# bacchus-snu/bacchus-gpu-controller

Hardware: AMD Instinct MI355X
Metric: reconcile p99 (ms) + admission p50 (ms); CR apply→Ready/sec on 8×MI355X node (higher is better)
Workload: dtype none

## Files before the change

native/apiserver/server.cc:

```cpp
#include "apiserver/server.h"

#include <algorithm>
#include <array>
#include <atomic>
#include <chrono>
#include <condition_variable>
#include <deque>
#include <functional>
#include <iterator>
#include <mutex>
#include <optional>
#include <regex>
#include <set>
#include <sstream>
#include <thread>
#include <unordered_map>
#include <unordered_set>

#include <openssl/crypto.h>

#include "apiserver/fieldset.h"
#include "core/crypto.h"
#include "core/http.h"
#include "core/json_patch.h"
#include "core/log.h"
#include "core/metrics.h"
#include "core/process.h"
#include "core/stall.h"
#include "core/trace.h"
#include "core/net.h"
#include "core/yaml.h"
#include "crd/schema.h"
#include "kube/leader.h"
#include "kube/quantity.h"
#include "kube/resource.h"

namespace bgc::apiserver {

using json::Value;
using kube::ResourceType;

namespace {


struct StatusError : std::runtime_error {
  int code;
  std::string reason;
  Value details;
  StatusError(int c, std::string r, const std::string& msg, Value d = {})
      : std::runtime_error(msg), code(c), reason(std::move(r)), details(std::move(d)) {}
};

Value status_body(int code, const std::string& reason, const std::string& message, const Value& details = {}) {
  Value s = Value::object({{"kind", "Status"}, {"apiVersion", "v1"}, {"metadata", Value::object()},
                           {"status", code < 400 ? "Success" : "Failure"}, {"message", message},
                           {"reason", reason}});
  if (!details.is_null()) s["details"] = details;
  s["code"] = code;
  return s;
}

std::string resource_ref(const ResourceType& rt) {
  return rt.group.empty() ? rt.plural : rt.plural + "." + rt.group;
}

StatusError not_found(const ResourceType& rt, const std::string& name) {
  return StatusError(404, "NotFound", resource_ref(rt) + " \"" + name + "\" not found",
                     Value::object({{"name", name}, {"group", rt.group}, {"kind", rt.plural}}));
}

StatusError already_exists(const ResourceType& rt, const std::string& name) {
  return StatusError(409, "AlreadyExists", resource_ref(rt) + " \"" + name + "\" already exists",
                     Value::object({{"name", name}, {"group", rt.group}, {"kind", rt.plural}}));
}

StatusError conflict(const ResourceType& rt, const std::string& name) {
  return StatusError(409, "Conflict",
                     "Operation cannot be fulfilled on " + resource_ref(rt) + " \"" + name +
                         "\": the object has been modified; please apply your changes to the latest version and try again",
                     Value::object({{"name", name}, {"group", rt.group}, {"kind", rt.plural}}));
}

StatusError invalid(const ResourceType& rt, const std::string& name, const std::string& msg) {
  return StatusError(422, "Invalid", rt.kind + "." + rt.group + " \"" + name + "\" is invalid: " + msg,
                     Value::object({{"name", name}, {"group", rt.group}, {"kind", rt.kind}}));
}

std::string now_rfc3339() {
  std::string s = kube::rfc3339_micro_now();
  return s.substr(0, 19) + "Z";
}

bool dns1123_label(const std::string& s) {
  if (s.empty() || s.size() > 63) return false;
  for (size_t i = 0; i < s.size(); ++i) {
    char c = s[i];
    bool ok = (c >= 'a' && c <= 'z') || (c >= '0' && c <= '9') || (c == '-' && i != 0 && i + 1 != s.size());
    if (!ok) return false;
  }
  return true;
}

bool dns1123_subdomain(const std::string& s) {
  if (s.empty() || s.size() > 253) return false;
  size_t start = 0;
  while (true) {
    size_t dot = s.find('.', start);
    std::string part = s.substr(start, dot == std::string::npos ? std::string::npos : dot - start);
    if (!dns1123_label(part)) return false;
    if (dot == std::string::npos) return true;
    start = dot + 1;
  }
}


struct Requirement {
  std::string key;
  std::string op;
  std::vector<std::string> values;
};

std::string trim(std::string s) {
  while (!s.empty() && s.front() == ' ') s.erase(0, 1);
  while (!s.empty() && s.back() == ' ') s.pop_back();
  return s;
}

std::vector<Requirement> parse_selector(const std::string& sel) {
  std::vector<Requirement> out;
  std::vector<std::string> parts;
  int depth = 0;
  std::string cur;
  for (char c : sel) {
    if (c == '(') ++depth;
    if (c == ')') --depth;
    if (c == ',' && depth == 0) {
      parts.push_back(cur);
      cur.clear();
    } else {
      cur.push_back(c);
    }
  }
  if (!cur.empty()) parts.push_back(cur);
  for (auto p : parts) {
    p = trim(p);
    if (p.empty()) continue;
    Requirement r;
    size_t pos;
    if (p[0] == '!') {
      r.key = trim(p.substr(1));
      r.op = "!exists";
    } else if ((pos = p.find(" notin ")) != std::string::npos || (pos = p.find(" in ")) != std::string::npos) {
      bool notin = p.compare(pos, 7, " notin ") == 0;
      r.key = trim(p.substr(0, pos));
      r.op = notin ? "notin" : "in";
      size_t lp = p.find('('), rp = p.rfind(')');
      if (lp == std::string::npos || rp == std::string::npos) throw StatusError(400, "BadRequest", "invalid selector: " + p);
      std::string inner = p.substr(lp + 1, rp - lp - 1);
      std::stringstream ss(inner);
      std::string v;
      while (std::getline(ss, v, ',')) r.values.push_back(trim(v));
    } else if ((pos = p.find("!=")) != std::string::npos) {
      r.key = trim(p.substr(0, pos));
      r.op = "!=";
      r.values.push_back(trim(p.substr(pos + 2)));
    } else if ((pos = p.find("==")) != std::string::npos) {
      r.key = trim(p.substr(0, pos));
      r.op = "=";
      r.values.push_back(trim(p.substr(pos + 2)));
    } else if ((pos = p.find('=')) != std::string::npos) {
      r.key = trim(p.substr(0, pos));
      r.op = "=";
      r.values.push_back(trim(p.substr(pos + 1)));
    } else {
      r.key = p;
      r.op = "exists";
    }
    out.push_back(r);
  }
  return out;
}

bool selector_matches(const std::vector<Requirement>& reqs, const Value& obj) {
  const Value& labels = obj.get("metadata").get("labels");
  for (const auto& r : reqs) {
    const Value* v = labels.find(r.key);
    bool has = v && v->is_string();
    std::string val = has ? v->as_string() : "";
    if (r.op == "exists" && !has) return false;
    if (r.op == "!exists" && has) return false;
    if (r.op == "=" && (!has || val != r.values[0])) return false;
    if (r.op == "!=" && has && val == r.values[0]) return false;
    if (r.op == "in" && (!has || std::find(r.values.begin(), r.values.end(), val) == r.values.end())) return false;
    if (r.op == "notin" && has && std::find(r.values.begin(), r.values.end(), val) != r.values.end()) return false;
  }
  return true;
}

struct FieldFilter {
  std::string name, ns;
  std::string name_prefix;
  bool name_ok(std::string_view n) const {
    return (name.empty() || n == name) && (name_prefix.empty() || n.substr(0, name_prefix.size()) == name_prefix);
  }
};

FieldFilter parse_field_selector(const std::string& s) {
  FieldFilter f;
  std::stringstream ss(s);
  std::string part;
  while (std::getline(ss, part, ',')) {
    size_t eq = part.find('=');
    if (eq == std::string::npos) continue;
    std::string k = trim(part.substr(0, eq));
    std::string v = trim(part.substr(part[eq + 1] == '=' ? eq + 2 : eq + 1));
    if (k == "metadata.name") f.name = v;
    else if (k == "metadata.namespace") f.ns = v;
    else if (k == "kube-lite.test/name-prefix") f.name_prefix = v;
  }
  return f;
}


struct UserInfo {
  std::string username;
  std::string uid;
  std::vector<std::string> groups;
  bool is_admin() const { return std::find(groups.begin(), groups.end(), "system:masters") != groups.end(); }
  Value to_json() const {
    Value g = Value::array();
    for (auto& x : groups) g.push_back(x);
    Value v = Value::object({{"username", username}});
    if (!uid.empty()) v["uid"] = uid;
    v["groups"] = g;
    return v;
  }
};

struct TypeStore;

struct TypeInfo {
  ResourceType rt;
  std::shared_ptr<const Value> schema;
  bool custom = false;
  std::shared_ptr<TypeStore> store;
  std::string key() const { return rt.group + "/" + rt.version + "/" + rt.plural; }
};

struct ManagerEntry {
  std::string operation;
  std::string api_version;
  std::string time;
  std::string subresource;
  FieldSet fields;
  bool operator==(const ManagerEntry& o) const {
    return operation == o.operation && fields == o.fields && subresource == o.subresource;
  }
};
using Managers = std::map<std::string, ManagerEntry>;

inline const std::shared_ptr<const Managers>& no_managers() {
  static const std::shared_ptr<const Managers> empty = std::make_shared<const Managers>();
  return empty;
}

struct Stored {
  std::shared_ptr<const Value> obj;
  uint64_t rv = 0;
  std::weak_ptr<const std::string> line;
  std::shared_ptr<const Managers> managers = no_managers();
};

bool wants_metadata(const http::Request& req) {
  const std::string* a = req.headers.get("Accept");
  return a && a->find("as=PartialObjectMetadata") != std::string::npos;
}

void dump_partial_metadata(const Value& obj, std::string& out) {
  out += "{\"kind\":\"PartialObjectMetadata\",\"apiVersion\":\"meta.k8s.io/v1\",\"metadata\":";
  obj.get("metadata").dump_to(out);
  out += "}";
}

std::string partial_metadata_line(const std::string& line) {
  std::string_view body(line);
  while (!body.empty() && (body.back() == '\n' || body.back() == '\r')) body.remove_suffix(1);
  const std::string_view type = json::raw_member(body, "type");
  const std::string_view md = json::raw_member(json::raw_member(body, "object"), "metadata");
  std::string out;
  out.reserve(md.size() + 128);
  out += "{\"type\":";
  out.append(type.data(), type.size());
  out += ",\"object\":{\"kind\":\"PartialObjectMetadata\",\"apiVersion\":\"meta.k8s.io/v1\",\"metadata\":";
  if (md.empty()) out += "{}";
  else out.append(md.data(), md.size());
  out += "}}\n";
  return out;
}

enum class View : uint8_t { AsIs, Added, Deleted };

struct EventRec {
  uint64_t rv;
  std::string type_key;
  std::string ns;
  std::shared_ptr<const Value> meta;
  std::shared_ptr<const std::string> line;
  struct Transitions {
    std::shared_ptr<const Value> prev_meta;
    std::shared_ptr<const std::string> prev_line;
    std::once_flag added_once, deleted_once;
    std::string added, added_meta, deleted, deleted_meta;
  };
  std::unique_ptr<Transitions> tr;
  const std::string& metadata_line() const {
    std::call_once(meta_once_, [this] { meta_line_ = partial_metadata_line(*line); });
    return meta_line_;
  }
  const std::string& line_as(View v, bool meta_only) const {
    if (v == View::AsIs || !tr) return meta_only ? metadata_line() : *line;
    Transitions& t = *tr;
    if (v == View::Added) {
      std::call_once(t.added_once, [&] {
        t.added = retyped_line(*line, "ADDED");
        t.added_meta = partial_metadata_line(t.added);
      });
      return meta_only ? t.added_meta : t.added;
    }
    std::call_once(t.deleted_once, [&] {
      t.deleted = deleted_from_prev();
      t.deleted_meta = partial_metadata_line(t.deleted);
    });
    return meta_only ? t.deleted_meta : t.deleted;
  }

 private:
  static std::string retyped_line(const std::string& l, const char* type) {
    const std::string_view t = json::raw_member(l, "type");
    std::string out;
    if (t.empty()) return l;
    out.reserve(l.size() + 8);
    out.append(l, 0, static_cast<size_t>(t.data() - l.data()));
    out += '"';
    out += type;
    out += '"';
    out.append(t.data() + t.size(), l.data() + l.size());
    return out;
  }
  std::string deleted_from_prev() const {
    std::string_view prev(*tr->prev_line);
    while (!prev.empty() && (prev.back() == '\n' || prev.back() == '\r')) prev.remove_suffix(1);
    const std::string_view obj = json::raw_member(prev, "object");
    const std::string_view old_rv = json::raw_member(json::raw_member(obj, "metadata"), "resourceVersion");
    const std::string_view new_rv =
        json::raw_member(json::raw_member(json::raw_member(*line, "object"), "metadata"), "resourceVersion");
    std::string out = "{\"type\":\"DELETED\",\"object\":";
    if (old_rv.empty()) {
      out.append(obj.data(), obj.size());
    } else {
      out.append(obj.data(), static_cast<size_t>(old_rv.data() - obj.data()));
      out.append(new_rv.data(), new_rv.size());
      out.append(old_rv.data() + old_rv.size(), obj.data() + obj.size());
    }
    out += "}\n";
    return out;
  }
  mutable std::once_flag meta_once_;
  mutable std::string meta_line_;
};

struct QueuedEvent {
  std::shared_ptr<const EventRec> e;
  View view = View::AsIs;
};

std::shared_ptr<const Value> filter_view(const Value& obj) {
  const Value& m = obj.get("metadata");
  Value meta = Value::object({{"name", m.get("name")}});
  if (m.contains("labels")) meta["labels"] = m.get("labels");
  return std::make_shared<const Value>(Value::object({{"metadata", std::move(meta)}}));
}

struct WatchSub {
  std::string type_key;
  std::string ns;
  std::vector<Requirement> sel;
  FieldFilter fields;
  std::mutex m;
  std::condition_variable cv;
  std::deque<QueuedEvent> q;
  bool closed = false;
  bool overflow = false;

  void close() {
    {
      std::lock_guard<std::mutex> g(m);
      closed = true;
    }
    cv.notify_one();
  }
};

class RwLock {
 public:
  RwLock() {
    const char* kind = std::getenv("BGC_KL_RWLOCK");
    mutex_only_ = !kind || (std::string(kind) != "writer" && std::string(kind) != "reader");
    pthread_rwlockattr_t a;
    pthread_rwlockattr_init(&a);
    pthread_rwlockattr_setkind_np(&a, kind && std::string(kind) == "reader" ? PTHREAD_RWLOCK_PREFER_READER_NP
                                                                           : PTHREAD_RWLOCK_PREFER_WRITER_NONRECURSIVE_NP);
    pthread_rwlock_init(&l_, &a);
    pthread_rwlockattr_destroy(&a);
  }
  ~RwLock() { pthread_rwlock_destroy(&l_); }
  RwLock(const RwLock&) = delete;
  RwLock& operator=(const RwLock&) = delete;
  void lock() {
    if (mutex_only_) m_.lock();
    else pthread_rwlock_wrlock(&l_);
  }
  bool try_lock() { return mutex_only_ ? m_.try_lock() : pthread_rwlock_trywrlock(&l_) == 0; }
  void unlock() {
    if (mutex_only_) m_.unlock();
    else pthread_rwlock_unlock(&l_);
  }
  void lock_shared() {
    if (mutex_only_) m_.lock();
    else pthread_rwlock_rdlock(&l_);
  }
  bool try_lock_shared() { return mutex_only_ ? m_.try_lock() : pthread_rwlock_tryrdlock(&l_) == 0; }
  void unlock_shared() { unlock(); }

 private:
  pthread_rwlock_t l_;
  std::mutex m_;
  bool mutex_only_ = false;
};

thread_local std::vector<std::shared_ptr<WatchSub>> t_pending_wakeups;
thread_local std::vector<std::shared_ptr<const EventRec>> t_retired_events;

inline void flush_watch_wakeups() {
  for (auto& w : t_pending_wakeups) w->cv.notify_one();
  t_pending_wakeups.clear();
  t_retired_events.clear();
}

struct LockStats {
  std::atomic<uint64_t> acquisitions{0}, shared{0}, contended{0}, wait_ns{0}, hold_ns{0};
};

class StoreLock {
 public:
  StoreLock(RwLock& m, LockStats& st, LockStats* also = nullptr) : m_(m), st_(st), also_(also) {
    if (!m_.try_lock()) {
      int64_t t0 = metrics::now_ns();
      m_.lock();
      const auto waited = static_cast<uint64_t>(metrics::now_ns() - t0);
      st_.contended.fetch_add(1, std::memory_order_relaxed);
      st_.wait_ns.fetch_add(waited, std::memory_order_relaxed);
      if (also_) {
        also_->contended.fetch_add(1, std::memory_order_relaxed);
        also_->wait_ns.fetch_add(waited, std::memory_order_relaxed);
      }
    }
    t_acq_ = metrics::now_ns();
  }
  ~StoreLock() {
    const auto held = static_cast<uint64_t>(metrics::now_ns() - t_acq_);
    st_.acquisitions.fetch_add(1, std::memory_order_relaxed);
    st_.hold_ns.fetch_add(held, std::memory_order_relaxed);
    if (also_) {
      also_->acquisitions.fetch_add(1, std::memory_order_relaxed);
      also_->hold_ns.fetch_add(held, std::memory_order_relaxed);
    }
    m_.unlock();
    flush_watch_wakeups();
  }
  StoreLock(const StoreLock&) = delete;
  StoreLock& operator=(const StoreLock&) = delete;

 private:
  RwLock& m_;
  LockStats& st_;
  LockStats* also_;
  int64_t t_acq_ = 0;
};

class SharedStoreLock {
 public:
  SharedStoreLock(RwLock& m, LockStats& st) : m_(m) {
    if (!m_.try_lock_shared()) {
      int64_t t0 = metrics::now_ns();
      m_.lock_shared();
      st.contended.fetch_add(1, std::memory_order_relaxed);
      st.wait_ns.fetch_add(static_cast<uint64_t>(metrics::now_ns() - t0), std::memory_order_relaxed);
    }
    st.shared.fetch_add(1, std::memory_order_relaxed);
  }
  ~SharedStoreLock() { m_.unlock_shared(); }
  SharedStoreLock(const SharedStoreLock&) = delete;
  SharedStoreLock& operator=(const SharedStoreLock&) = delete;

 private:
  RwLock& m_;
};

struct TypeStore {
  struct Shard {
    RwLock mu;
    std::unordered_map<std::string, Stored> objs;
  };
  class Shards {
   public:
    explicit Shards(size_t n) : n_(std::max<size_t>(1, n)), p_(new Shard[n_]) {}
    Shard* begin() { return p_.get(); }
    Shard* end() { return p_.get() + n_; }
    std::reverse_iterator<Shard*> rbegin() { return std::reverse_iterator<Shard*>(end()); }
    std::reverse_iterator<Shard*> rend() { return std::reverse_iterator<Shard*>(begin()); }
    size_t size() const { return n_; }
    Shard& operator[](size_t i) { return p_[i]; }

   private:
    size_t n_;
    std::unique_ptr<Shard[]> p_;
  };
  explicit TypeStore(size_t n_shards) : shards(n_shards) {}
  Shards shards;
  Shard& shard(const std::string& key) {
    return shards.size() == 1 ? shards[0] : shards[std::hash<std::string>{}(key) % shards.size()];
  }
  RwLock seq;
  std::atomic<uint64_t> version{0};
  LockStats stats;
  LockStats seq_stats;
  std::deque<std::shared_ptr<const EventRec>> history;
  uint64_t compacted_rv = 0;
  std::mutex watches_mu;
  std::set<std::shared_ptr<WatchSub>> watches;
};

class AllShards {
 public:
  AllShards(TypeStore& ts, bool exclusive) : ts_(ts), exclusive_(exclusive) {
    for (auto& sh : ts_.shards) {
      if (exclusive_) {
        if (!sh.mu.try_lock()) {
          const int64_t t0 = metrics::now_ns();
          sh.mu.lock();
          ts_.stats.contended.fetch_add(1, std::memory_order_relaxed);
          ts_.stats.wait_ns.fetch_add(static_cast<uint64_t>(metrics::now_ns() - t0), std::memory_order_relaxed);
        }
      } else if (!sh.mu.try_lock_shared()) {
        const int64_t t0 = metrics::now_ns();
        sh.mu.lock_shared();
        ts_.stats.contended.fetch_add(1, std::memory_order_relaxed);
        ts_.stats.wait_ns.fetch_add(static_cast<uint64_t>(metrics::now_ns() - t0), std::memory_order_relaxed);
      }
    }
    ts_.stats.acquisitions.fetch_add(1, std::memory_order_relaxed);
  }
  ~AllShards() {
    for (auto it = ts_.shards.rbegin(); it != ts_.shards.rend(); ++it) {
      if (exclusive_) it->mu.unlock();
      else it->mu.unlock_shared();
    }
    flush_watch_wakeups();
  }
  AllShards(const AllShards&) = delete;
  AllShards& operator=(const AllShards&) = delete;

 private:
  TypeStore& ts_;
  bool exclusive_;
};

struct FaultRule {
  std::string method;
  std::regex path;
  std::string path_src;
  int status = 0;
  int retry_after_s = -1;
  int delay_ms = 0;
  int hold_ms = 0;
  int remaining = -1;
  bool reset = false;
  std::string message;
};

struct ParsedPath {
  TypeInfo* ti = nullptr;
  std::string ns;
  std::string name;
  std::string sub;
  bool collection = false;
};

thread_local std::string t_trace_tag;
thread_local std::string t_trace_name;

void trace_step(const std::string& name, const char* step) {
  if (!t_trace_tag.empty()) trace::mark(name, t_trace_tag + step);
}

struct WriteResult {
  std::shared_ptr<const Value> obj;
  int code = 200;
  std::shared_ptr<const std::string> line;
  std::string_view body() const {
    static const std::string kPrefixEnd = ",\"object\":";
    if (!line) return {};
    size_t at = line->find(kPrefixEnd);
    if (at == std::string::npos || line->size() < at + kPrefixEnd.size() + 2) return {};
    at += kPrefixEnd.size();
    return std::string_view(*line).substr(at, line->size() - at - 2);
  }
};

std::string obj_key(const ResourceType& rt, const std::string& ns, const std::string& name) { return rt.key(ns, name); }

}


struct ApiServer::Impl {
  Options opts;
  std::unique_ptr<http::Server> server;

  RwLock types_mu;
  std::map<std::string, TypeInfo> types;
  std::atomic<uint64_t> rv{1000};
  std::mutex index_mu;
  std::unordered_map<std::string, std::pair<std::string, std::string>> by_uid;
  using Ref = std::pair<std::string, std::string>;
  struct RefHash {
    size_t operator()(const Ref& r) const { return std::hash<std::string>{}(r.first) * 31 + std::hash<std::string>{}(r.second); }
  };
  std::unordered_map<std::string, std::unordered_set<Ref, RefHash>> by_owner;
  std::unordered_map<std::string, std::unordered_set<Ref, RefHash>> by_namespace;

  struct GcItem {
    bool is_namespace = false;
    std::string id;
    bool finish_namespace = false;
  };
  std::mutex gc_mu;
  std::condition_variable gc_cv;
  std::deque<GcItem> gc_queue;
  bool gc_stop = false;
  std::atomic<uint64_t> gc_collected{0};
  std::vector<std::thread> gc_threads;

  std::unordered_map<std::string, UserInfo> tokens;

  std::mutex fault_mu;
  std::vector<FaultRule> faults;

  struct ListSnapshot {
    uint64_t rv = 0;
    std::vector<std::shared_ptr<const Value>> items;
    std::chrono::steady_clock::time_point expires;
  };
  std::mutex list_mu;
  std::map<uint64_t, ListSnapshot> list_snapshots;
  uint64_t next_list_id = 1;
  std::atomic<uint64_t> list_pages{0};

  static constexpr uint64_t kRvMask = 0x5bd1e9955bd1e995ULL;
  std::string rv_str(uint64_t v) const {
    if (!opts.opaque_rv) return std::to_string(v);
    static const char* digits = "0123456789abcdefghijklmnopqrstuvwxyz";
    uint64_t x = v ^ kRvMask;
    std::string out;
    do {
      out.insert(out.begin(), digits[x % 36]);
      x /= 36;
    } while (x);
    return "kl." + out;
  }
  bool parse_rv(const std::string& s, uint64_t* v) const {
    if (!opts.opaque_rv) {
      if (s.empty() || s.find_first_not_of("0123456789") != std::string::npos) return false;
      *v = std::strtoull(s.c_str(), nullptr, 10);
      return true;
    }
    if (s.rfind("kl.", 0) != 0 || s.size() < 4) return false;
    uint64_t x = 0;
    for (size_t i = 3; i < s.size(); ++i) {
      const char c = s[i];
      int d = c >= '0' && c <= '9' ? c - '0' : c >= 'a' && c <= 'z' ? c - 'a' + 10 : -1;
      if (d < 0) return false;
      x = x * 36 + static_cast<uint64_t>(d);
    }
    *v = x ^ kRvMask;
    return true;
  }

  std::mutex hook_mu;
  struct FastHook {
    std::shared_ptr<const Value> cfg;
    std::shared_ptr<http::Client> client;
    std::string path;
  };
  std::map<const Value*, FastHook> hook_fast;
  std::map<std::string, std::shared_ptr<http::Client>> hook_clients;
  std::atomic<bool> webhook_h2{false};
  std::atomic<int64_t> write_latency_us{0};
  std::atomic<int> watch_coalesce_us{0};

  std::atomic<uint64_t> requests{0};
  std::atomic<uint64_t> faults_hit{0};
  LockStats types_stats;

  explicit Impl(Options o) : opts(std::move(o)) {
    if (const char* e = std::getenv("BGC_KL_STORE_SHARDS"); e && *e) opts.store_shards = std::max(1, std::atoi(e));
    watch_coalesce_us = opts.watch_coalesce_us;
    if (const char* e = std::getenv("BGC_KL_H2_CALLER_READS"); e && *e) opts.webhook_h2_caller_reads = std::string(e) != "0";
    webhook_h2 = opts.webhook_http2;
    write_latency_us = opts.write_latency_us;
    for (const ResourceType* rt : kube::types::builtin()) {
      TypeInfo ti;
      ti.rt = *rt;
      ti.store = std::make_shared<TypeStore>(opts.store_shards);
      types[ti.key()] = ti;
    }
    if (!opts.token_file.empty()) load_tokens(opts.token_file);
    const TypeInfo& ns_ti = types.at(kube::types::Namespace.group + "/" + kube::types::Namespace.version + "/" +
                                     kube::types::Namespace.plural);
    for (const char* name : {"default", "kube-system", "kube-public", "kube-node-lease"}) {
      const uint64_t v = ++rv;
      Value ns = Value::object(
          {{"apiVersion", "v1"}, {"kind", "Namespace"},
           {"metadata", Value::object({{"name", name}, {"uid", crypto::uuid_v4()}, {"creationTimestamp", now_rfc3339()},
                                       {"resourceVersion", rv_str(v)}})},
           {"spec", Value::object({{"finalizers", Value::array({Value("kubernetes")})}})},
           {"status", Value::object({{"phase", "Active"}})}});
      Stored st;
      st.obj = std::make_shared<const Value>(std::move(ns));
      st.rv = v;
      ns_ti.store->shard(obj_key(ns_ti.rt, "", name)).objs[obj_key(ns_ti.rt, "", name)] = std::move(st);
    }
    for (int i = 0; i < std::max(1, opts.gc_workers); ++i) gc_threads.emplace_back([this] {
      gc_loop();
      OPENSSL_thread_stop();
    });
  }

  ~Impl() {
    {
      std::lock_guard<std::mutex> g(gc_mu);
      gc_stop = true;
    }
    gc_cv.notify_all();
    for (auto& t : gc_threads) t.join();
  }

  template <typename F>
  void for_each_store(F f) {
    std::vector<std::pair<std::string, std::shared_ptr<TypeStore>>> stores;
    {
      SharedStoreLock lk(types_mu, types_stats);
      for (auto& [k, ti] : types) stores.emplace_back(k, ti.store);
    }
    for (auto& [k, st] : stores) f(k, *st);
  }

  TypeInfo* type_by_key(const std::string& key) {
    SharedStoreLock lk(types_mu, types_stats);
    auto it = types.find(key);
    return it == types.end() ? nullptr : &it->second;
  }

  void load_tokens(const std::string& path) {
    std::stringstream ss(net::read_file(path));
    std::string line;
    while (std::getline(ss, line)) {
      if (line.empty() || line[0] == '#') continue;
      std::vector<std::string> cols;
      std::string cur;
      bool q = false;
      for (char c : line) {
        if (c == '"') {
          q = !q;
          continue;
        }
        if (c == ',' && !q) {
          cols.push_back(cur);
          cur.clear();
          continue;
        }
        cur.push_back(c);
      }
      cols.push_back(cur);
      if (cols.size() < 2) continue;
      UserInfo u;
      u.username = cols[1];
      if (cols.size() > 2) u.uid = cols[2];
      if (cols.size() > 3 && !cols[3].empty()) {
        std::stringstream gs(cols[3]);
        std::string g;
        while (std::getline(gs, g, ',')) u.groups.push_back(g);
      }
      u.groups.push_back("system:authenticated");
      tokens[cols[0]] = u;
    }
  }

  UserInfo authenticate(const http::Request& req) {
    UserInfo u;
    std::string auth = req.headers.get_or("Authorization");
    if (auth.rfind("Bearer ", 0) == 0) {
      auto it = tokens.find(auth.substr(7));
      if (it == tokens.end()) throw StatusError(401, "Unauthorized", "Unauthorized");
      u = it->second;
    } else if (!req.peer_cn.empty()) {
      u.username = req.peer_cn;
      u.groups = req.peer_orgs;
      u.groups.push_back("system:authenticated");
    } else if (opts.anonymous_admin) {
      u.username = "system:admin";
      u.groups = {"system:masters", "system:authenticated"};
    } else {
      throw StatusError(401, "Unauthorized", "Unauthorized");
    }
    if (const std::string* imp = req.headers.get("Impersonate-User")) {
      if (!u.is_admin()) {
        throw StatusError(403, "Forbidden", "users \"" + *imp + "\" is forbidden: User \"" + u.username +
                                                "\" cannot impersonate resource \"users\" in API group \"\" at the cluster scope");
      }
      UserInfo imp_u;
      imp_u.username = *imp;
      for (const auto& kv : req.headers.items()) {
        std::string lk = kv.first;
        for (auto& c : lk) c = static_cast<char>(std::tolower(static_cast<unsigned char>(c)));
        if (lk == "impersonate-group") {
          std::stringstream gs(kv.second);
          std::string g;
          while (std::getline(gs, g, ',')) {
            if (!trim(g).empty()) imp_u.groups.push_back(trim(g));
          }
        }
      }
      imp_u.groups.push_back("system:authenticated");
      u = imp_u;
    }
    return u;
  }

  TypeInfo* find_type(const std::string& group, const std::string& version, const std::string& plural) {
    auto it = types.find(group + "/" + version + "/" + plural);
    return it == types.end() ? nullptr : &it->second;
  }

  bool parse_path(const std::string& path, ParsedPath& out, std::string& group, std::string& version,
                  std::vector<std::string>& rest) {
    std::vector<std::string> segs;
    std::stringstream ss(path);
    std::string s;
    while (std::getline(ss, s, '/')) {
      if (!s.empty()) segs.push_back(s);
    }
    size_t i = 0;
    if (segs.size() >= 2 && segs[0] == "api") {
      group = "";
      version = segs[1];
      i = 2;
    } else if (segs.size() >= 3 && segs[0] == "apis") {
      group = segs[1];
      version = segs[2];
      i = 3;
    } else {
      return false;
    }
    rest.assign(segs.begin() + static_cast<long>(i), segs.end());
    if (rest.empty()) return false;
    SharedStoreLock lk(types_mu, types_stats);
    if (rest[0] == "namespaces" && rest.size() >= 3) {
      TypeInfo* ti = find_type(group, version, rest[2]);
      if (ti && ti->rt.namespaced) {
        out.ti = ti;
        out.ns = rest[1];
        out.collection = rest.size() == 3;
        if (rest.size() >= 4) out.name = rest[3];
        if (rest.size() >= 5) out.sub = rest[4];
        return true;
      }
    }
    TypeInfo* ti = find_type(group, version, rest[0]);
    if (!ti) throw StatusError(404, "NotFound", "the server could not find the requested resource");
    out.ti = ti;
    out.collection = rest.size() == 1;
    if (rest.size() >= 2) out.name = rest[1];
    if (rest.size() >= 3) out.sub = rest[2];
    return true;
  }

  struct PreparedEvent {
    std::string head, tail;
    bool ok = false;
    std::shared_ptr<const Value> filter;
    std::shared_ptr<EventRec> rec;
  };

  std::shared_ptr<const std::string> emit_locked(const TypeInfo& ti, const std::string& ns, uint64_t ev_rv,
                                                 std::string line, std::shared_ptr<const Value> filter,
                                                 std::shared_ptr<EventRec> rec) {
    TypeStore& st = *ti.store;
    st.version.fetch_add(1, std::memory_order_release);
    if (!rec) rec = std::make_shared<EventRec>();
    rec->rv = ev_rv;
    rec->type_key = ti.key();
    rec->ns = ns;
    rec->meta = std::move(filter);
    rec->line = std::make_shared<const std::string>(std::move(line));
    st.history.push_back(rec);
    while (st.history.size() > opts.history_limit) {
      st.compacted_rv = st.history.front()->rv;
      t_retired_events.push_back(std::move(st.history.front()));
      st.history.pop_front();
    }
    const std::string& name = rec->meta->get("metadata").get_string("name");
    std::lock_guard<std::mutex> wg(st.watches_mu);
    for (const auto& w : st.watches) {
      if (!w->ns.empty() && w->ns != ns) continue;
      if (!w->fields.name_ok(name)) continue;
      View view;
      if (!view_for(w->sel, *rec, &view)) continue;
      {
        std::lock_guard<std::mutex> g(w->m);
        if (w->q.size() > 100000) w->overflow = true;
        else w->q.push_back({rec, view});
      }
      t_pending_wakeups.push_back(w);
    }
    return rec->line;
  }

  static bool view_for(const std::vector<Requirement>& sel, const EventRec& e, View* view) {
    *view = View::AsIs;
    if (sel.empty()) return true;
    const bool now_in = selector_matches(sel, *e.meta);
    if (!e.tr) return now_in;
    const bool was_in = selector_matches(sel, *e.tr->prev_meta);
    if (now_in && !was_in) *view = View::Added;
    else if (!now_in && was_in) *view = View::Deleted;
    return now_in || was_in;
  }

  struct HookMatch {
    std::string name;
    std::shared_ptr<const Value> cfg;
    const Value* hook;
  };
  std::mutex hook_match_mu;
  uint64_t hook_match_version = ~uint64_t{0};
  std::unordered_map<std::string, std::vector<HookMatch>> hook_match_cache;

  std::vector<HookMatch> matching_webhooks(const TypeInfo& ti, const std::string& sub, const std::string& op) {
    TypeInfo* mwc = type_by_key(kube::types::MutatingWebhookConfiguration.group + "/v1/mutatingwebhookconfigurations");
    if (!mwc) return {};
    const std::string cache_key = ti.key() + "|" + sub + "|" + op;
    {
      std::lock_guard<std::mutex> g(hook_match_mu);
      if (hook_match_version == mwc->store->version.load(std::memory_order_acquire)) {
        auto it = hook_match_cache.find(cache_key);
        if (it != hook_match_cache.end()) return it->second;
      }
    }
    std::vector<HookMatch> out;
    AllShards lk(*mwc->store, false);
    const uint64_t version = mwc->store->version.load(std::memory_order_acquire);
    std::string res = ti.rt.plural + (sub.empty() ? "" : "/" + sub);
    for (auto& sh : mwc->store->shards)
    for (auto& kv : sh.objs) {
      for (const auto& hook : kv.second.obj->get("webhooks").items()) {
        for (const auto& rule : hook.get("rules").items()) {
          auto contains = [](const Value& arr, const std::string& v) {
            for (const auto& x : arr.items()) {
              if (x.is_string() && (x.as_string() == "*" || x.as_string() == v)) return true;
            }
            return false;
          };
          bool res_ok = false;
          for (const auto& r : rule.get("resources").items()) {
            std::string rs = r.as_string();
            if (rs == res || rs == "*/*" || (rs == "*" && sub.empty()) ||
                (sub.size() && rs == "*/" + sub) || (rs == ti.rt.plural + "/*")) {
              res_ok = true;
            }
          }
          if (contains(rule.get("apiGroups"), ti.rt.group) && contains(rule.get("apiVersions"), ti.rt.version) &&
              contains(rule.get("operations"), op) && res_ok) {
            out.push_back({hook.get_string("name"), kv.second.obj, &hook});
            break;
          }
        }
      }
    }
    {
      std::lock_guard<std::mutex> g(hook_match_mu);
      if (hook_match_version != version) {
        hook_match_cache.clear();
        hook_match_version = version;
      }
      hook_match_cache[cache_key] = out;
    }
    return out;
  }

  std::shared_ptr<http::Client> hook_client(const HookMatch& hm, std::string& path_out) {
    {
      std::lock_guard<std::mutex> lk(hook_mu);
      auto it = hook_fast.find(hm.hook);
      if (it != hook_fast.end()) {
        path_out = it->second.path;
        return it->second.client;
      }
    }
    auto c = hook_client_slow(*hm.hook, path_out);
    std::lock_guard<std::mutex> lk(hook_mu);
    if (hook_fast.size() > 256) hook_fast.clear();
    hook_fast[hm.hook] = {hm.cfg, c, path_out};
    return c;
  }

  std::shared_ptr<http::Client> hook_client_slow(const Value& hook, std::string& path_out) {
    const Value& cc = hook.get("clientConfig");
    std::string ca = cc.get_string("caBundle");
    std::string base, server_name;
    if (cc.get("url").is_string()) {
      http::Url u = http::parse_url(cc.get_string("url"));
      base = u.scheme + "://" + u.host + ":" + std::to_string(u.port);
      path_out = u.path.empty() ? "/" : u.path;
    } else {
      const Value& svc = cc.get("service");
      std::string ns = svc.get_string("namespace"), name = svc.get_string("name");
      int port = svc.get("port").is_int() ? static_cast<int>(svc.get("port").as_int()) : 443;
      path_out = svc.get_string("path", "/");
      server_name = name + "." + ns + ".svc";
      auto ov = opts.service_overrides.find(ns + "/" + name);
      std::string hostport = ov != opts.service_overrides.end() ? ov->second : server_name + ":" + std::to_string(port);
      base = "https://" + hostport;
    }
    std::string key = base + "|" + server_name + "|" + crypto::sha256_hex(ca);
    std::lock_guard<std::mutex> lk(hook_mu);
    auto it = hook_clients.find(key);
    if (it != hook_clients.end()) return it->second;
    http::ClientOptions o;
    o.base_url = base;
    o.tls_server_name = server_name;
    o.http2 = webhook_h2.load();
    o.h2_connections = opts.webhook_h2_connections;
    o.h2_caller_reads = opts.webhook_h2_caller_reads;
    if (base.rfind("https", 0) == 0) {
      o.tls = net::TlsContext::client(ca.empty() ? "" : crypto::base64_decode(ca), false);
    }
    auto c = std::make_shared<http::Client>(o);
    hook_clients[key] = c;
    return c;
  }

  void call_webhooks(const TypeInfo& ti, const std::string& sub, const std::string& op, const std::string& ns,
                     const std::string& name, Value* obj, const Value* old, const UserInfo& user) {
    auto hooks = matching_webhooks(ti, sub, op);
    if (hooks.empty()) return;
    static auto& hist = metrics::Registry::global().histogram("kl_webhook_duration_seconds", "Webhook callout latency");
    static auto& calls = metrics::Registry::global().counter("kl_webhook_calls_total", "Webhook callouts (any outcome)");
    static auto& ring = [] () -> metrics::SampleLog& {
      auto& r = metrics::Registry::global().samples("webhook");
      r.link("kl_webhook_calls_total", &calls);
      return r;
    }();
    for (const auto& hm : hooks) {
      const Value& hook = *hm.hook;
      std::string fail_policy = hook.get_string("failurePolicy", "Fail");
      int timeout_s = hook.get("timeoutSeconds").is_int() ? static_cast<int>(hook.get("timeoutSeconds").as_int()) : 10;
      std::string uid = crypto::uuid_v4();
      const std::string opts_kind = op == "CREATE" ? "CreateOptions" : op == "DELETE" ? "DeleteOptions" : "UpdateOptions";
      const std::string gvk = "{\"group\":" + json::quote(ti.rt.group) + ",\"version\":" + json::quote(ti.rt.version) +
                              ",\"kind\":" + json::quote(ti.rt.kind) + "}";
      const std::string gvr = "{\"group\":" + json::quote(ti.rt.group) + ",\"version\":" + json::quote(ti.rt.version) +
                              ",\"resource\":" + json::quote(ti.rt.plural) + "}";
      std::string body;
      body.reserve(1024 + (obj ? 2048 : 0) + (old ? 2048 : 0));
      body += "{\"kind\":\"AdmissionReview\",\"apiVersion\":\"admission.k8s.io/v1\",\"request\":{\"uid\":";
      body += json::quote(uid);
      body += ",\"kind\":" + gvk + ",\"resource\":" + gvr;
      if (!sub.empty()) body += ",\"subResource\":" + json::quote(sub);
      body += ",\"requestKind\":" + gvk + ",\"requestResource\":" + gvr;
      if (!sub.empty()) body += ",\"requestSubResource\":" + json::quote(sub);
      body += ",\"name\":" + json::quote(name);
      if (!ns.empty()) body += ",\"namespace\":" + json::quote(ns);
      body += ",\"operation\":" + json::quote(op);
      body += ",\"userInfo\":";
      user.to_json().dump_to(body);
      body += ",\"object\":";
      if (obj) obj->dump_to(body);
      else body += "null";
      body += ",\"oldObject\":";
      if (old) old->dump_to(body);
      else body += "null";
      body += ",\"dryRun\":false,\"options\":{\"kind\":" + json::quote(opts_kind) +
              ",\"apiVersion\":\"meta.k8s.io/v1\"}}}";
      std::string err;
      Value resp_review;
      int64_t t0 = metrics::now_ns();
      try {
        std::string path;
        auto client = hook_client(hm, path);
        http::Headers h;
        h.set("Content-Type", "application/json");
        h.set("Accept", "application/json");
        http::Response r = client->request("POST", path + "?timeout=" + std::to_string(timeout_s) + "s",
                                           body, &h, timeout_s * 1000);
        if (r.status != 200) {
          err = "expected webhook response status code 200, got " + std::to_string(r.status) + ": " + r.body;
        } else if (!json::try_parse(r.body, resp_review, &err)) {
          err = "failed to parse webhook response: " + err;
        }
      } catch (const std::exception& e) {
        err = e.what();
      }
      double secs = static_cast<double>(metrics::now_ns() - t0) * 1e-9;
      hist.observe(secs);
      ring.add(secs, &calls);
      const Value& resp = resp_review.get("response");
      if (err.empty() && !resp.is_object()) err = "webhook response was absent";
      if (err.empty() && resp.get_string("uid") != uid) {
        err = "expected response.uid=\"" + uid + "\", got \"" + resp.get_string("uid") + "\"";
      }
      if (!err.empty()) {
        if (fail_policy == "Ignore") {
          LOG_WARN("apiserver") << "failed calling webhook " << hm.name << " (ignored): " << err;
          continue;
        }
        throw StatusError(500, "InternalError",
                          "Internal error occurred: failed calling webhook \"" + hm.name + "\": " + err);
      }
      if (!resp.get("allowed").is_bool() || !resp.get("allowed").as_bool()) {
        const Value& st = resp.get("status");
        int code = st.get("code").is_int() ? static_cast<int>(st.get("code").as_int()) : 0;
        if (code < 400) code = 400;
        std::string reason = st.get_string("reason", code == 403 ? "Forbidden" : "BadRequest");
        std::string msg = "admission webhook \"" + hm.name + "\" denied the request";
        std::string m = st.get_string("message");
        msg += m.empty() ? " without explanation" : ": " + m;
        throw StatusError(code, reason, msg);
      }
      if (resp.get("patch").is_string() && obj) {
        if (resp.get_string("patchType", "JSONPatch") != "JSONPatch") {
          throw StatusError(500, "InternalError", "unsupported patchType from webhook " + hm.name);
        }
        Value patch;
        std::string perr;
        if (!json::try_parse(crypto::base64_decode(resp.get_string("patch")), patch, &perr)) {
          throw StatusError(500, "InternalError", "invalid patch from webhook " + hm.name + ": " + perr);
        }
        try {
          json::apply_patch(*obj, patch);
        } catch (const std::exception& e) {
          throw StatusError(500, "InternalError",
                            "Internal error occurred: failed calling webhook \"" + hm.name + "\": " + e.what());
        }
      }
    }
  }

  void validate_object(const TypeInfo& ti, const std::string& name, const std::string& ns, const Value& obj) {
    const Value& meta = obj.get("metadata");
    if (ti.rt.plural == "namespaces") {
      if (!dns1123_label(name)) {
        throw invalid(ti.rt, name, "metadata.name: Invalid value: \"" + name +
                                       "\": a lowercase RFC 1123 label must consist of lower case alphanumeric characters or '-', and must start and end with an alphanumeric character");
      }
    } else if (!dns1123_subdomain(name)) {
      throw invalid(ti.rt, name, "metadata.name: Invalid value: \"" + name +
                                     "\": a lowercase RFC 1123 subdomain must consist of lower case alphanumeric characters, '-' or '.', and must start and end with an alphanumeric character");
    }
    if (meta.get("namespace").is_string() && ti.rt.namespaced && meta.get_string("namespace") != ns) {
      throw StatusError(400, "BadRequest", "the namespace of the provided object does not match the namespace sent on the request");
    }
    for (const auto& ref : meta.get("ownerReferences").items()) {
      for (const char* f : {"apiVersion", "kind", "name", "uid"}) {
        if (!ref.get(f).is_string() || ref.get_string(f).empty()) {
          throw invalid(ti.rt, name, std::string("metadata.ownerReferences.") + f + ": Invalid value: \"\": " + f +
                                         " must not be empty");
        }
      }
    }
    if (ti.rt.plural == "rolebindings" || ti.rt.plural == "clusterrolebindings") {
      if (!obj.get("roleRef").is_object()) throw invalid(ti.rt, name, "roleRef: Required value");
    }
    std::shared_ptr<const Value> schema = std::atomic_load(&ti.schema);
    if (opts.validate_schema && ti.custom && schema && schema->is_object()) {
      auto errs = crd::validate(obj, *schema);
      if (!errs.empty()) {
        std::string msg;
        for (size_t i = 0; i < errs.size() && i < 5; ++i) {
          if (i) msg += ", ";
          const auto& e = errs[i];
          if (e.kind == "required") msg += e.path + ": Required value";
          else msg += e.path + ": Invalid value: " + e.detail;
        }
        throw invalid(ti.rt, name, msg);
      }
    }
  }

  void register_crd(const Value& crd) {
    const Value& spec = crd.get("spec");
    std::string group = spec.get_string("group");
    const Value& names = spec.get("names");
    bool namespaced = spec.get_string("scope") == "Namespaced";
    StoreLock lk(types_mu, types_stats);
    for (const auto& v : spec.get("versions").items()) {
      if (v.get("served").is_bool() && !v.get("served").as_bool()) continue;
      TypeInfo ti;
      ti.rt.group = group;
      ti.rt.version = v.get_string("name");
      ti.rt.kind = names.get_string("kind");
      ti.rt.plural = names.get_string("plural");
      ti.rt.namespaced = namespaced;
      ti.rt.has_status = v.get("subresources").get("status").is_object();
      auto schema = std::make_shared<const Value>(v.get("schema").get("openAPIV3Schema"));
      ti.custom = true;
      auto it = types.find(ti.key());
      if (it != types.end()) {
        std::atomic_store(&it->second.schema, schema);
        continue;
      }
      ti.schema = schema;
      ti.store = std::make_shared<TypeStore>(opts.store_shards);
      types[ti.key()] = ti;
    }
  }

  enum class NsPhase { Missing, Active, Terminating };
  NsPhase namespace_phase(const std::string& ns) {
    TypeInfo* nti = type_by_key(kube::types::Namespace.group + "/v1/namespaces");
    if (!nti) return NsPhase::Missing;
    const std::string key = obj_key(nti->rt, "", ns);
    auto& sh = nti->store->shard(key);
    SharedStoreLock lk(sh.mu, nti->store->stats);
    auto it = sh.objs.find(key);
    if (it == sh.objs.end()) return NsPhase::Missing;
    if (!it->second.obj->get("metadata").contains("deletionTimestamp")) return NsPhase::Active;
    return opts.namespace_termination ? NsPhase::Terminating : NsPhase::Missing;
  }

  static bool is_core_namespaces(const TypeInfo& ti) { return ti.rt.plural == "namespaces" && ti.rt.group.empty(); }

  std::shared_ptr<const Value> terminate_namespace_locked(const TypeInfo& ti, const std::string& name, Stored& cur) {
    Value obj = *cur.obj;
    obj["metadata"]["deletionTimestamp"] = now_rfc3339();
    obj["metadata"]["deletionGracePeriodSeconds"] = 0;
    obj["status"]["phase"] = "Terminating";
    auto ptr = commit_locked(ti, "", name, std::move(obj), *cur.managers, &cur);
    std::lock_guard<std::mutex> g(gc_mu);
    gc_queue.push_back({true, name, true});
    gc_cv.notify_one();
    return ptr;
  }

  void finish_namespace(const std::string& name) {
    TypeInfo* nti = type_by_key(kube::types::Namespace.group + "/v1/namespaces");
    if (!nti) return;
    const std::string key = obj_key(nti->rt, "", name);
    auto& sh = nti->store->shard(key);
    StoreLock lk(sh.mu, nti->store->stats);
    auto it = sh.objs.find(key);
    if (it == sh.objs.end() || !it->second.obj->get("metadata").contains("deletionTimestamp")) return;
    if (it->second.obj->get("metadata").get("finalizers").empty()) {
      erase_locked(*nti, "", name);
      return;
    }
    Value obj = *it->second.obj;
    if (obj.get("spec").get("finalizers").empty()) return;
    obj["spec"]["finalizers"] = Value::array();
    commit_locked(*nti, "", name, std::move(obj), *it->second.managers, &it->second);
  }

  static void render_managed(Value& obj, const Managers& m, const std::string& api_version) {
    Value arr = Value::array();
    for (const auto& [key, e] : m) {
      if (e.fields.empty()) continue;
      std::string mgr = key.substr(0, key.find('\x1f'));
      Value ent = Value::object({{"manager", mgr}, {"operation", e.operation},
                                 {"apiVersion", e.api_version.empty() ? api_version : e.api_version},
                                 {"time", e.time}, {"fieldsType", "FieldsV1"}, {"fieldsV1", fields_v1(e.fields)}});
      if (!e.subresource.empty()) ent["subresource"] = e.subresource;
      arr.push_back(std::move(ent));
    }
    if (arr.empty()) obj["metadata"].erase("managedFields");
    else obj["metadata"]["managedFields"] = std::move(arr);
  }

  static bool same_content(const Value& a, const Value& b) {
    if (!a.is_object() || !b.is_object()) return a == b;
    auto volatile_key = [](const std::string& k) { return k == "managedFields" || k == "resourceVersion"; };
    auto count = [&](const Value& v, bool meta) {
      size_t n = 0;
      for (const auto& k : v.keys()) n += (meta && volatile_key(k)) ? 0 : 1;
      return n;
    };
    if (a.size() != b.size()) return false;
    for (size_t i = 0; i < a.keys().size(); ++i) {
      const std::string& k = a.keys()[i];
      const Value* bv = b.find(k);
      if (!bv) return false;
      const Value& av = a.values()[i];
      if (k != "metadata") {
        if (!(av == *bv)) return false;
        continue;
      }
      if (!av.is_object() || !bv->is_object()) {
        if (!(av == *bv)) return false;
        continue;
      }
      if (count(av, true) != count(*bv, true)) return false;
      for (size_t j = 0; j < av.keys().size(); ++j) {
        const std::string& mk = av.keys()[j];
        if (volatile_key(mk)) continue;
        const Value* bm = bv->find(mk);
        if (!bm || !(av.values()[j] == *bm)) return false;
      }
    }
    return true;
  }

  static bool spec_changed(const Value& a, const Value& b) {
    if (!a.is_object() || !b.is_object()) return !(a == b);
    auto skip = [](const std::string& k) { return k == "metadata" || k == "status"; };
    size_t na = 0, nb = 0;
    for (size_t i = 0; i < a.keys().size(); ++i) {
      const std::string& k = a.keys()[i];
      if (skip(k)) continue;
      ++na;
      const Value* bv = b.find(k);
      if (!bv || !(a.values()[i] == *bv)) return true;
    }
    for (const auto& k : b.keys()) nb += skip(k) ? 0 : 1;
    return na != nb;
  }

  static void attribute_update(Managers& m, const std::string& manager, const Value& before, const Value& after,
                               bool status_write, const std::string& api_version) {
    FieldSet changed, removed;
    if (status_write) diff_member_leaves(before, after, "status", changed, removed);
    else diff_leaves(before, after, changed, removed);
    for (auto& [name, e] : m) {
      for (const auto& p : changed) e.fields.erase(p);
      for (const auto& p : removed) e.fields.erase(p);
    }
    if (!changed.empty()) {
      auto& e = m[status_write ? manager + "\x1fstatus" : manager];
      if (e.operation.empty()) {
        e.operation = "Update";
        e.api_version = api_version;
      }
      if (e.operation == "Apply") {
        e.operation = "Update";
      }
      e.time = now_rfc3339();
      if (status_write) e.subresource = "status";
      for (const auto& p : changed) e.fields.insert(p);
    }
    for (auto it = m.begin(); it != m.end();) {
      if (it->second.fields.empty()) it = m.erase(it);
      else ++it;
    }
  }

  static const std::string& rv_placeholder() {
    static const std::string p = "\x01rv\x01";
    return p;
  }
  static PreparedEvent prepare_commit(Value& obj, const Managers& managers, const std::string& api_version,
                                      const char* type) {
    obj["metadata"]["resourceVersion"] = rv_placeholder();
    render_managed(obj, managers, api_version);
    std::string line = std::string("{\"type\":\"") + type + "\",\"object\":";
    obj.dump_to(line);
    line += "}\n";
    static const std::string needle = "\"resourceVersion\":" + Value(rv_placeholder()).dump();
    PreparedEvent pe;
    pe.filter = filter_view(obj);
    pe.rec = std::make_shared<EventRec>();
    size_t pos = line.find(needle);
    if (pos == std::string::npos) return pe;
    pe.head.assign(line, 0, pos);
    pe.head += "\"resourceVersion\":\"";
    pe.tail.assign(line, pos + needle.size() - 1, std::string::npos);
    pe.ok = true;
    return pe;
  }

  std::shared_ptr<const Value> commit_locked(const TypeInfo& ti, const std::string& ns, const std::string& name,
                                            Value obj, Managers managers, const Stored* prev,
                                            const PreparedEvent* pe = nullptr, bool* dangling = nullptr,
                                            std::shared_ptr<const std::string>* line_out = nullptr) {
    TypeStore& ts = *ti.store;
    PreparedEvent local;
    if (!pe || !pe->ok) {
      local = prepare_commit(obj, managers, ti.rt.api_version(), prev ? "MODIFIED" : "ADDED");
      pe = &local;
    }
    std::string key = obj_key(ti.rt, ns, name);
    Ref ref{ti.key(), key};
    {
      std::lock_guard<std::mutex> ig(index_mu);
      if (prev) unindex_owners_locked(*prev->obj, ref);
      by_uid[obj.get("metadata").get_string("uid")] = ref;
      const Value& owners = obj.get("metadata").get("ownerReferences");
      for (const auto& r : owners.items()) by_owner[r.get_string("uid")].insert(ref);
      if (ti.rt.namespaced) by_namespace[ns].insert(ref);
      if (dangling && !prev && !owners.empty()) {
        bool alive = false;
        for (const auto& r : owners.items()) alive = alive || by_uid.count(r.get_string("uid")) > 0;
        *dangling = !alive;
      }
    }
    std::shared_ptr<EventRec> rec = pe->rec ? pe->rec : std::make_shared<EventRec>();
    if (prev && opts.selector_transitions &&
        prev->obj->get("metadata").get("labels") != obj.get("metadata").get("labels")) {
      auto t = std::make_unique<EventRec::Transitions>();
      t->prev_meta = filter_view(*prev->obj);
      if (auto held = prev->line.lock()) {
        t->prev_line = std::move(held);
      } else {
        std::string l = "{\"type\":\"MODIFIED\",\"object\":";
        prev->obj->dump_to(l);
        l += "}\n";
        t->prev_line = std::make_shared<const std::string>(std::move(l));
      }
      rec->tr = std::move(t);
    }
    uint64_t new_rv;
    std::string digits;
    std::shared_ptr<const std::string> line;
    {
      StoreLock sl(ts.seq, ts.seq_stats);
      new_rv = ++rv;
      digits = rv_str(new_rv);
      std::string preline;
      if (pe->ok) {
        preline.reserve(pe->head.size() + digits.size() + pe->tail.size());
        preline += pe->head;
        preline += digits;
        preline += pe->tail;
      } else {
        obj["metadata"]["resourceVersion"] = digits;
        preline = std::string("{\"type\":\"") + (prev ? "MODIFIED" : "ADDED") + "\",\"object\":";
        obj.dump_to(preline);
        preline += "}\n";
      }
      line = emit_locked(ti, ns, new_rv, std::move(preline), pe->filter ? pe->filter : filter_view(obj), std::move(rec));
    }
    obj["metadata"]["resourceVersion"] = digits;
    auto ptr = std::make_shared<const Value>(std::move(obj));
    Stored s;
    s.obj = ptr;
    s.rv = new_rv;
    s.managers = std::make_shared<const Managers>(std::move(managers));
    s.line = line;
    ts.shard(key).objs[key] = std::move(s);
    if (line_out) *line_out = std::move(line);
    return ptr;
  }

  void unindex_owners_locked(const Value& obj, const Ref& ref) {
    for (const auto& r : obj.get("metadata").get("ownerReferences").items()) {
      auto it = by_owner.find(r.get_string("uid"));
      if (it == by_owner.end()) continue;
      it->second.erase(ref);
      if (it->second.empty()) by_owner.erase(it);
    }
  }

  void erase_locked(const TypeInfo& ti, const std::string& ns, const std::string& name) {
    TypeStore& ts = *ti.store;
    std::string key = obj_key(ti.rt, ns, name);
    auto& b = ts.shard(key).objs;
    auto it = b.find(key);
    if (it == b.end()) return;
    std::shared_ptr<const Value> ptr = it->second.obj;
    std::string line = "{\"type\":\"DELETED\",\"object\":";
    const size_t obj_at = line.size();
    static const std::string kObjectKey = ",\"object\":";
    const std::shared_ptr<const std::string> held = it->second.line.lock();
    const std::string* committed = held.get();
    const size_t at = committed ? committed->find(kObjectKey) : std::string::npos;
    if (at != std::string::npos && committed->size() >= at + kObjectKey.size() + 2) {
      line.append(*committed, at + kObjectKey.size(), committed->size() - (at + kObjectKey.size()) - 2);
    } else {
      ptr->dump_to(line);
    }
    line += "}\n";
    const std::string old_rv = "\"resourceVersion\":" + json::quote(ptr->get("metadata").get_string("resourceVersion"));
    const size_t pos = line.find(old_rv, obj_at);
    auto filter = filter_view(*ptr);
    std::string uid = ptr->get("metadata").get_string("uid");
    Ref ref{ti.key(), key};
    bool has_dependents;
    {
      std::lock_guard<std::mutex> ig(index_mu);
      by_uid.erase(uid);
      unindex_owners_locked(*ptr, ref);
      if (ti.rt.namespaced) {
        auto nit = by_namespace.find(ns);
        if (nit != by_namespace.end()) {
          nit->second.erase(ref);
          if (nit->second.empty()) by_namespace.erase(nit);
        }
      }
      has_dependents = by_owner.count(uid) > 0;
    }
    uint64_t new_rv;
    {
      StoreLock sl(ts.seq, ts.seq_stats);
      new_rv = ++rv;
      const std::string digits = rv_str(new_rv);
      if (pos != std::string::npos) {
        line.replace(pos, old_rv.size(), "\"resourceVersion\":\"" + digits + "\"");
      } else {
        Value final_obj = *ptr;
        final_obj["metadata"]["resourceVersion"] = digits;
        line = "{\"type\":\"DELETED\",\"object\":";
        final_obj.dump_to(line);
        line += "}\n";
      }
      emit_locked(ti, ns, new_rv, std::move(line), std::move(filter), nullptr);
    }
    b.erase(it);
    bool is_ns = ti.rt.plural == "namespaces" && ti.rt.group.empty();
    if (has_dependents || is_ns) {
      std::lock_guard<std::mutex> g(gc_mu);
      if (has_dependents) gc_queue.push_back({false, uid});
      if (is_ns) gc_queue.push_back({true, name});
      gc_cv.notify_one();
    }
  }

  void gc_loop() {
    while (true) {
      GcItem item;
      {
        std::unique_lock<std::mutex> g(gc_mu);
        gc_cv.wait(g, [&] { return gc_stop || !gc_queue.empty(); });
        if (gc_stop) return;
        item = std::move(gc_queue.front());
        gc_queue.pop_front();
      }
      std::vector<Ref> victims;
      {
        std::lock_guard<std::mutex> ig(index_mu);
        auto& idx = item.is_namespace ? by_namespace : by_owner;
        auto it = idx.find(item.id);
        if (it != idx.end()) victims.assign(it->second.begin(), it->second.end());
      }
      for (const auto& v : victims) {
        TypeInfo* vti = type_by_key(v.first);
        if (!vti) continue;
        auto& vsh = vti->store->shard(v.second);
        StoreLock lk(vsh.mu, vti->store->stats);
        auto it = vsh.objs.find(v.second);
        if (it == vsh.objs.end()) continue;
        const Value& meta = it->second.obj->get("metadata");
        if (!item.is_namespace) {
          bool alive = false;
          {
            std::lock_guard<std::mutex> ig(index_mu);
            for (const auto& r : meta.get("ownerReferences").items()) alive = alive || by_uid.count(r.get_string("uid")) > 0;
          }
          if (alive) continue;
        }
        std::string vns = meta.get_string("namespace"), vname = meta.get_string("name");
        if (is_core_namespaces(*vti) && opts.namespace_termination) {
          if (!meta.contains("deletionTimestamp")) terminate_namespace_locked(*vti, vname, it->second);
          continue;
        }
        erase_locked(*vti, vns, vname);
        gc_collected.fetch_add(1, std::memory_order_relaxed);
      }
      if (item.finish_namespace) finish_namespace(item.id);
    }
  }

  static void canonicalize_quantities(const TypeInfo& ti, Value& obj) {
    if (ti.custom || (ti.rt.plural != "resourcequotas" && ti.rt.plural != "nodes")) return;
    auto fix = [](Value* m) {
      if (!m || !m->is_object()) return;
      for (Value& v : m->items_mut()) {
        std::string text;
        if (v.is_string()) text = v.as_string();
        else if (v.is_int()) text = v.dump();
        else continue;
        if (auto c = kube::canonical_quantity(text)) {
          if (!v.is_string() || *c != text) v = Value(std::move(*c));
        }
      }
    };
    auto sub = [](Value& o, const char* k) { return o.is_object() ? o.find_mut(k) : nullptr; };
    Value* spec = sub(obj, "spec");
    Value* status = sub(obj, "status");
    if (ti.rt.plural == "resourcequotas") {
      if (spec) fix(sub(*spec, "hard"));
      if (status) {
        fix(sub(*status, "hard"));
        fix(sub(*status, "used"));
      }
    } else if (status) {
      fix(sub(*status, "capacity"));
      fix(sub(*status, "allocatable"));
    }
  }

  using Compute = std::function<std::pair<Value, Managers>(const Stored* cur)>;

  WriteResult write(TypeInfo& ti, const std::string& ns, const std::string& name, const std::string& sub,
                    const UserInfo& user, const Compute& compute, bool allow_create, bool is_status) {
    for (int attempt = 0; attempt < 8; ++attempt) {
      Stored cur_copy;
      bool exists = false;
      const std::string key = obj_key(ti.rt, ns, name);
      auto& sh = ti.store->shard(key);
      {
        SharedStoreLock lk(sh.mu, ti.store->stats);
        auto it = sh.objs.find(key);
        if (it != sh.objs.end()) {
          cur_copy = it->second;
          exists = true;
        }
      }
      if (!exists && !allow_create) throw not_found(ti.rt, name);
      auto [obj, managers] = compute(exists ? &cur_copy : nullptr);
      canonicalize_quantities(ti, obj);
      std::string op = exists ? "UPDATE" : "CREATE";
      if (!exists && ti.rt.namespaced) {
        const NsPhase phase = namespace_phase(ns);
        if (phase == NsPhase::Missing) {
          throw StatusError(404, "NotFound", "namespaces \"" + ns + "\" not found",
                            Value::object({{"name", ns}, {"kind", "namespaces"}}));
        }
        if (phase == NsPhase::Terminating) {
          throw StatusError(
              403, "Forbidden",
              ti.rt.plural + " \"" + name + "\" is forbidden: unable to create new content in namespace " + ns +
                  " because it is being terminated",
              Value::object({{"name", name}, {"kind", ti.rt.plural},
                             {"causes", Value::array({Value::object({{"reason", "NamespaceTerminating"},
                                                                     {"message", "namespace " + ns + " is being terminated"},
                                                                     {"field", "metadata.namespace"}})})}}));
        }
      }
      if (exists && same_content(obj, *cur_copy.obj) && managers == *cur_copy.managers) {
        return {cur_copy.obj, 200, nullptr};
      }
      trace_step(name, ".hook0");
      call_webhooks(ti, sub, op, ns, name, &obj, exists ? cur_copy.obj.get() : nullptr, user);
      trace_step(name, ".hook1");
      obj["metadata"]["name"] = name;
      if (ti.rt.namespaced) obj["metadata"]["namespace"] = ns;
      else obj["metadata"].erase("namespace");
      canonicalize_quantities(ti, obj);
      validate_object(ti, name, ns, obj);
      if (exists && same_content(obj, *cur_copy.obj) && managers == *cur_copy.managers) {
        return {cur_copy.obj, 200, nullptr};
      }
      if (exists && spec_changed(*cur_copy.obj, obj)) {
        int64_t gen = cur_copy.obj->get("metadata").get("generation").is_int()
                          ? cur_copy.obj->get("metadata").get("generation").as_int()
                          : 1;
        obj["metadata"]["generation"] = gen + 1;
      }
      PreparedEvent pe = prepare_commit(obj, managers, ti.rt.api_version(), exists ? "MODIFIED" : "ADDED");
      StoreLock lk(sh.mu, ti.store->stats);
      auto it = sh.objs.find(key);
      bool now_exists = it != sh.objs.end();
      if (now_exists != exists || (exists && it->second.rv != cur_copy.rv)) continue;
      if (exists) {
        if (obj.get("metadata").contains("deletionTimestamp") && obj.get("metadata").get("finalizers").empty() &&
            !(is_core_namespaces(ti) && opts.namespace_termination && !obj.get("spec").get("finalizers").empty())) {
          erase_locked(ti, ns, name);
          return {cur_copy.obj, 200, nullptr};
        }
        (void)is_status;
        WriteResult wr;
        trace_step(name, ".commit");
        wr.obj = commit_locked(ti, ns, name, std::move(obj), std::move(managers), &it->second, &pe, nullptr, &wr.line);
        return wr;
      }
      if (ti.rt.plural == "customresourcedefinitions") register_crd(obj);
      bool dangling = false;
      std::shared_ptr<const std::string> line;
      trace_step(name, ".commit");
      auto created = commit_locked(ti, ns, name, std::move(obj), std::move(managers), nullptr, &pe, &dangling, &line);
      if (dangling) erase_locked(ti, ns, name);
      WriteResult wr;
      wr.obj = created;
      wr.code = 201;
      wr.line = std::move(line);
      return wr;
    }
    throw conflict(ti.rt, name);
  }

  void init_new(const TypeInfo& ti, Value& obj, const std::string& ns, const std::string& name) {
    obj["apiVersion"] = ti.rt.api_version();
    obj["kind"] = ti.rt.kind;
    Value& meta = obj["metadata"];
    meta["name"] = name;
    if (ti.rt.namespaced) meta["namespace"] = ns;
    meta["uid"] = crypto::uuid_v4();
    meta["creationTimestamp"] = now_rfc3339();
    meta["generation"] = 1;
    meta.erase("resourceVersion");
    meta.erase("deletionTimestamp");
    meta.erase("managedFields");
    if (ti.rt.has_status && ti.custom) obj.erase("status");
    if (ti.rt.plural == "namespaces" && ti.rt.group.empty()) {
      obj["spec"] = Value::object({{"finalizers", Value::array({"kubernetes"})}});
      obj["status"] = Value::object({{"phase", "Active"}});
    }
  }

  static void carry_meta(Value& obj, const Value& cur) {
    const Value& cm = cur.get("metadata");
    Value& m = obj["metadata"];
    for (const char* f : {"uid", "creationTimestamp", "generation", "deletionTimestamp"}) {
      if (cm.contains(f)) m[f] = cm.get(f);
      else m.erase(f);
    }
    obj["apiVersion"] = cur.get("apiVersion");
    obj["kind"] = cur.get("kind");
  }

  std::string field_manager(const http::Request& req, const std::string& dflt) {
    std::string fm = req.query_param("fieldManager");
    if (!fm.empty()) return fm;
    std::string ua = req.headers.get_or("User-Agent", dflt);
    size_t slash = ua.find('/');
    return slash == std::string::npos ? ua : ua.substr(0, slash);
  }

  Value parse_body(const http::Request& req) {
    Value v;
    std::string err;
    std::string ct = req.headers.get_or("Content-Type");
    if (ct.find("yaml") != std::string::npos && !req.body.empty() && req.body[0] != '{') {
      try {
        return yaml::parse(req.body);
      } catch (const std::exception& e) {
        throw StatusError(400, "BadRequest", std::string("error decoding YAML: ") + e.what());
      }
    }
    if (!json::try_parse(req.body, v, &err)) throw StatusError(400, "BadRequest", "couldn't get version/kind; json parse error: " + err);
    return v;
  }

  void do_create(ParsedPath& p, const http::Request& req, const UserInfo& user, http::ResponseWriter& w) {
    Value body = parse_body(req);
    if (!body.is_object()) throw StatusError(400, "BadRequest", "object must be a JSON object");
    std::string name = body.get("metadata").get_string("name");
    if (name.empty()) {
      std::string gen = body.get("metadata").get_string("generateName");
      if (gen.empty()) throw invalid(p.ti->rt, "", "metadata.name: Required value: name or generateName is required");
      static const char* alnum = "bcdfghjklmnpqrstvwxz2456789";
      std::string rnd = crypto::random_bytes(5);
      name = gen;
      for (unsigned char c : rnd) name.push_back(alnum[c % 27]);
    }
    std::string manager = field_manager(req, "unknown");
    if (!t_trace_tag.empty()) t_trace_name = name;
    auto res = write(*p.ti, p.ns, name, "", user,
                     [&](const Stored* cur) -> std::pair<Value, Managers> {
                       if (cur) throw already_exists(p.ti->rt, name);
                       Value obj = body;
                       init_new(*p.ti, obj, p.ns, name);
                       Managers m;
                       attribute_update(m, manager, Value::object(), obj, false, p.ti->rt.api_version());
                       return {std::move(obj), std::move(m)};
                     },
                     true, false);
    {
      std::string_view b = res.body();
      if (!b.empty()) w.send_json(res.code, b);
      else w.send_json(res.code, res.obj->dump());
    }
  }

  void do_update(ParsedPath& p, const http::Request& req, const UserInfo& user, http::ResponseWriter& w) {
    Value body = parse_body(req);
    if (!body.is_object()) throw StatusError(400, "BadRequest", "object must be a JSON object");
    std::string bname = body.get("metadata").get_string("name");
    if (!bname.empty() && bname != p.name) {
      throw StatusError(400, "BadRequest", "the name of the object (" + bname +
                                               ") does not match the name on the URL (" + p.name + ")");
    }
    bool is_status = p.sub == "status";
    std::string manager = field_manager(req, "unknown");
    auto res = write(*p.ti, p.ns, p.name, p.sub, user,
                     [&](const Stored* cur) -> std::pair<Value, Managers> {
                       std::string want_rv = body.get("metadata").get_string("resourceVersion");
                       if (!want_rv.empty() && want_rv != cur->obj->get("metadata").get_string("resourceVersion")) {
                         throw conflict(p.ti->rt, p.name);
                       }
                       Value obj;
                       if (is_status) {
                         obj = *cur->obj;
                         if (body.contains("status")) obj["status"] = body.get("status");
                         else obj.erase("status");
                       } else {
                         obj = body;
                         carry_meta(obj, *cur->obj);
                         if (p.ti->rt.has_status) {
                           if (cur->obj->contains("status")) obj["status"] = cur->obj->get("status");
                           else obj.erase("status");
                         }
                       }
                       Managers m = *cur->managers;
                       attribute_update(m, manager, *cur->obj, obj, is_status, p.ti->rt.api_version());
                       return {std::move(obj), std::move(m)};
                     },
                     false, is_status);
    {
      std::string_view b = res.body();
      if (!b.empty()) w.send_json(res.code, b);
      else w.send_json(res.code, res.obj->dump());
    }
  }

  std::pair<Value, Managers> apply_ssa(const TypeInfo& ti, const Stored* cur, const Value& config,
                                       const std::string& manager_name, bool force, bool is_status,
                                       const std::string& ns, const std::string& name) {
    const std::string manager = is_status ? manager_name + "\x1fstatus" : manager_name;
    FieldSet cfg_fields = leaves(config, is_status);
    if (is_status) {
      FieldSet only;
      for (const auto& f : cfg_fields) {
        if (f == "/status" || f.rfind("/status/", 0) == 0) only.insert(f);
      }
      cfg_fields.swap(only);
    }
    Value live;
    Managers m;
    if (cur) {
      live = *cur->obj;
      m = *cur->managers;
    } else {
      live = Value::object();
      init_new(ti, live, ns, name);
    }
    std::vector<std::pair<std::string, std::string>> conflicts;
    for (const auto& f : cfg_fields) {
      const Value* want = get_path(config, f);
      const Value* have = get_path(live, f);
      for (auto& [other, e] : m) {
        if (other == manager || !e.fields.count(f)) continue;
        if (have && want && *have == *want) continue;
        conflicts.emplace_back(other, f);
      }
    }
    if (!conflicts.empty() && !force) {
      std::string msg = "Apply failed with " + std::to_string(conflicts.size()) + " conflict" +
                        (conflicts.size() > 1 ? "s" : "") + ": ";
      for (size_t i = 0; i < conflicts.size(); ++i) {
        if (i) msg += "; ";
        msg += "conflict with \"" + conflicts[i].first.substr(0, conflicts[i].first.find('\x1f')) + "\": " +
               display_path(conflicts[i].second);
      }
      throw StatusError(409, "Conflict", msg);
    }
    if (force) {
      for (const auto& [other, f] : conflicts) m[other].fields.erase(f);
    }
    if (auto it = m.find(manager); it != m.end()) {
      for (const auto& f : it->second.fields) {
        if (cfg_fields.count(f)) continue;
        bool other_owner = false;
        for (auto& [other, e] : m) {
          if (other != manager && e.fields.count(f)) other_owner = true;
        }
        if (!other_owner) remove_path(live, f);
      }
    }
    for (const auto& f : cfg_fields) {
      if (const Value* v = get_path(config, f)) set_path(live, f, *v);
    }
    auto& me = m[manager];
    me.operation = "Apply";
    me.api_version = ti.rt.api_version();
    me.time = now_rfc3339();
    me.subresource = is_status ? "status" : "";
    me.fields = cfg_fields;
    for (auto it = m.begin(); it != m.end();) {
      if (it->second.fields.empty()) it = m.erase(it);
      else ++it;
    }
    if (cur && ti.rt.has_status && !is_status) {
      if (cur->obj->contains("status")) live["status"] = cur->obj->get("status");
    }
    return {std::move(live), std::move(m)};
  }

  void do_patch(ParsedPath& p, const http::Request& req, const UserInfo& user, http::ResponseWriter& w) {
    std::string ct = req.headers.get_or("Content-Type");
    bool is_status = p.sub == "status";
    bool is_apply = ct.find("apply-patch") != std::string::npos;
    std::string manager = field_manager(req, is_apply ? "" : "unknown");
    if (is_apply && req.query_param("fieldManager").empty()) {
      throw StatusError(400, "BadRequest", "PatchOptions.meta.k8s.io \"\" is invalid: fieldManager: Required value: is required for apply patch");
    }
    Value patch = parse_body(req);
    bool force = req.query_param("force") == "true";
    auto res = write(*p.ti, p.ns, p.name, p.sub, user,
                     [&](const Stored* cur) -> std::pair<Value, Managers> {
                       if (is_apply) {
                         std::string pname = patch.get("metadata").get_string("name");
                         if (!pname.empty() && pname != p.name) {
                           throw StatusError(400, "BadRequest", "the name of the object (" + pname +
                                                                    ") does not match the name on the URL (" + p.name + ")");
                         }
                         return apply_ssa(*p.ti, cur, patch, manager, force, is_status, p.ns, p.name);
                       }
                       Value obj = *cur->obj;
                       try {
                         if (ct.find("json-patch") != std::string::npos) {
                           json::apply_patch(obj, patch);
                         } else {
                           json::apply_merge_patch(obj, patch);
                         }
                       } catch (const json::PatchError& e) {
                         throw StatusError(422, "Invalid", std::string("the server rejected our request due to an error in our request: ") + e.what());
                       }
                       std::string want_rv = obj.get("metadata").get_string("resourceVersion");
                       if (!want_rv.empty() && want_rv != cur->obj->get("metadata").get_string("resourceVersion")) {
                         throw conflict(p.ti->rt, p.name);
                       }
                       if (is_status) {
                         Value keep = *cur->obj;
                         if (obj.contains("status")) keep["status"] = obj.get("status");
                         else keep.erase("status");
                         obj = std::move(keep);
                       } else {
                         carry_meta(obj, *cur->obj);
                         if (p.ti->rt.has_status) {
                           if (cur->obj->contains("status")) obj["status"] = cur->obj->get("status");
                           else obj.erase("status");
                         }
                       }
                       Managers m = *cur->managers;
                       attribute_update(m, manager, *cur->obj, obj, is_status, p.ti->rt.api_version());
                       return {std::move(obj), std::move(m)};
                     },
                     is_apply, is_status);
    {
      std::string_view b = res.body();
      if (!b.empty()) w.send_json(res.code, b);
      else w.send_json(res.code, res.obj->dump());
    }
  }

  void do_delete(ParsedPath& p, const http::Request& req, const UserInfo& user, http::ResponseWriter& w) {
    std::shared_ptr<const Value> cur;
    const std::string key = obj_key(p.ti->rt, p.ns, p.name);
    auto& sh = p.ti->store->shard(key);
    {
      SharedStoreLock lk(sh.mu, p.ti->store->stats);
      auto it = sh.objs.find(key);
      if (it == sh.objs.end()) throw not_found(p.ti->rt, p.name);
      cur = it->second.obj;
    }
    trace_step(p.name, ".hook0");
    call_webhooks(*p.ti, "", "DELETE", p.ns, p.name, nullptr, cur.get(), user);
    trace_step(p.name, ".hook1");
    StoreLock lk(sh.mu, p.ti->store->stats);
    auto it = sh.objs.find(key);
    if (it == sh.objs.end()) throw not_found(p.ti->rt, p.name);
    const Value& meta = it->second.obj->get("metadata");
    if (is_core_namespaces(*p.ti) && opts.namespace_termination) {
      auto ptr = meta.contains("deletionTimestamp") ? it->second.obj
                                                    : terminate_namespace_locked(*p.ti, p.name, it->second);
      w.send_json(200, ptr->dump());
      return;
    }
    if (!meta.get("finalizers").empty()) {
      if (!meta.contains("deletionTimestamp")) {
        Value obj = *it->second.obj;
        obj["metadata"]["deletionTimestamp"] = now_rfc3339();
        obj["metadata"]["deletionGracePeriodSeconds"] = 0;
        auto ptr = commit_locked(*p.ti, p.ns, p.name, std::move(obj), *it->second.managers, &it->second);
        w.send_json(202, ptr->dump());
        return;
      }
      w.send_json(202, it->second.obj->dump());
      return;
    }
    erase_locked(*p.ti, p.ns, p.name);
    (void)req;
    w.send_json(200, status_body(200, "", "").dump());
  }

  void do_get(ParsedPath& p, http::ResponseWriter& w, bool meta_only = false) {
    std::shared_ptr<const Value> obj;
    {
      const std::string key = obj_key(p.ti->rt, p.ns, p.name);
      auto& sh = p.ti->store->shard(key);
      SharedStoreLock lk(sh.mu, p.ti->store->stats);
      auto it = sh.objs.find(key);
      if (it == sh.objs.end()) throw not_found(p.ti->rt, p.name);
      obj = it->second.obj;
    }
    if (meta_only) {
      std::string out;
      dump_partial_metadata(*obj, out);
      w.send_json(200, out);
      return;
    }
    w.send_json(200, obj->dump());
  }

  void do_list(ParsedPath& p, const http::Request& req, http::ResponseWriter& w) {
    const int64_t limit = req.has_query_param("limit") ? std::atoll(req.query_param("limit").c_str()) : 0;
    const std::string cont = req.query_param("continue");
    std::vector<std::shared_ptr<const Value>> items;
    uint64_t list_rv = 0;
    size_t offset = 0;
    uint64_t snap_id = 0;
    if (!cont.empty()) {
      const size_t dot = cont.find('.');
      snap_id = std::strtoull(cont.c_str(), nullptr, 10);
      offset = dot == std::string::npos ? 0 : std::strtoull(cont.c_str() + dot + 1, nullptr, 10);
      std::lock_guard<std::mutex> lk(list_mu);
      auto it = list_snapshots.find(snap_id);
      if (it == list_snapshots.end() || std::chrono::steady_clock::now() > it->second.expires) {
        if (it != list_snapshots.end()) list_snapshots.erase(it);
        throw StatusError(410, "Expired",
                          "The provided continue parameter is too old to display a consistent list result. You can "
                          "start a new list without the continue parameter.");
      }
      list_rv = it->second.rv;
      items = it->second.items;
    } else {
      auto sel = parse_selector(req.query_param("labelSelector"));
      auto ff = parse_field_selector(req.query_param("fieldSelector"));
      {
        AllShards lk(*p.ti->store, false);
        list_rv = rv.load();
        for (auto& sh : p.ti->store->shards)
        for (auto& [k, st] : sh.objs) {
          const Value& meta = st.obj->get("metadata");
          if (!p.ns.empty() && meta.get_string("namespace") != p.ns) continue;
          if (!ff.name_ok(meta.get_string("name"))) continue;
          if (!ff.ns.empty() && meta.get_string("namespace") != ff.ns) continue;
          if (!sel.empty() && !selector_matches(sel, *st.obj)) continue;
          items.push_back(st.obj);
        }
      }
      std::sort(items.begin(), items.end(), [](const auto& a, const auto& b) {
        const Value& ma = a->get("metadata");
        const Value& mb = b->get("metadata");
        return std::make_pair(ma.get_string("namespace"), ma.get_string("name")) <
               std::make_pair(mb.get_string("namespace"), mb.get_string("name"));
      });
    }
    size_t end = items.size();
    std::string next;
    if (limit > 0 && offset + static_cast<size_t>(limit) < items.size()) {
      end = offset + static_cast<size_t>(limit);
      std::lock_guard<std::mutex> lk(list_mu);
      if (snap_id == 0) {
        const auto now = std::chrono::steady_clock::now();
        for (auto it = list_snapshots.begin(); it != list_snapshots.end();) {
          it = now > it->second.expires ? list_snapshots.erase(it) : std::next(it);
        }
        snap_id = next_list_id++;
        list_snapshots[snap_id] = ListSnapshot{list_rv, items, now + std::chrono::milliseconds(opts.continue_ttl_ms)};
      }
      next = std::to_string(snap_id) + "." + std::to_string(end);
    } else if (snap_id != 0) {
      std::lock_guard<std::mutex> lk(list_mu);
      list_snapshots.erase(snap_id);
    }
    if (limit > 0) list_pages.fetch_add(1);
    const bool meta_only = wants_metadata(req);
    std::string out = meta_only ? std::string("{\"apiVersion\":\"meta.k8s.io/v1\",\"kind\":\"PartialObjectMetadataList\"")
                                : "{\"apiVersion\":" + json::quote(p.ti->rt.api_version()) + ",\"kind\":" +
                                      json::quote(p.ti->rt.kind + "List");
    out += ",\"metadata\":{\"resourceVersion\":\"" + rv_str(list_rv) + "\"";
    if (!next.empty()) {
      out += ",\"continue\":" + json::quote(next) +
             ",\"remainingItemCount\":" + std::to_string(items.size() - end);
    }
    out += "},\"items\":[";
    for (size_t i = offset; i < end; ++i) {
      if (i != offset) out.push_back(',');
      if (meta_only) dump_partial_metadata(*items[i], out);
      else items[i]->dump_to(out);
    }
    out += "]}";
    w.send_json(200, out);
  }

  void do_watch(ParsedPath& p, const http::Request& req, http::ResponseWriter& w) {
    auto subp = std::make_shared<WatchSub>();
    WatchSub& sub = *subp;
    sub.type_key = p.ti->key();
    sub.ns = p.ns;
    sub.sel = parse_selector(req.query_param("labelSelector"));
    sub.fields = parse_field_selector(req.query_param("fieldSelector"));
    if (!sub.fields.ns.empty()) sub.ns = sub.fields.ns;
    std::string rv_s = req.query_param("resourceVersion");
    const bool meta_only = wants_metadata(req);
    int timeout_s = opts.max_watch_seconds;
    if (req.has_query_param("timeoutSeconds")) timeout_s = std::min(timeout_s, std::atoi(req.query_param("timeoutSeconds").c_str()));
    bool bookmarks = req.query_param("allowWatchBookmarks") == "true";
    const std::string trace_watch = "kl.watch." + p.ti->rt.plural + "." + field_manager(req, "unknown") + ".sent";
    const std::string trace_written = trace_watch.substr(0, trace_watch.size() - 4) + "written";
    const std::string slow_write = "kw:" + p.ti->rt.plural + " write";
    set_thread_name("kw:" + p.ti->rt.plural);
    struct Rename {
      ~Rename() { set_thread_name("conn:apiserver"); }
    } rename;
    const bool send_initial = req.query_param("sendInitialEvents") == "true";
    if (send_initial && (!bookmarks || req.query_param("resourceVersionMatch") != "NotOlderThan")) {
      throw StatusError(422, "Invalid",
                        "sendInitialEvents requires allowWatchBookmarks=true and resourceVersionMatch=NotOlderThan");
    }
    uint64_t from = 0;
    if (!rv_s.empty() && rv_s != "0" && !parse_rv(rv_s, &from)) {
      throw StatusError(400, "BadRequest", "invalid resource version: " + rv_s);
    }
    std::vector<std::shared_ptr<const std::string>> initial;
    bool gone = false;
    TypeStore& ts = *p.ti->store;
    uint64_t compacted = 0;
    uint64_t initial_rv = 0;
    {
      const bool snapshot = rv_s.empty() || rv_s == "0" || send_initial;
      std::optional<AllShards> shards_lk;
      if (snapshot) shards_lk.emplace(ts, false);
      SharedStoreLock lk(ts.seq, ts.seq_stats);
      compacted = ts.compacted_rv;
      initial_rv = rv.load();
      if (snapshot) {
        for (auto& sh : ts.shards)
        for (auto& [k, st] : sh.objs) {
          const Value& meta = st.obj->get("metadata");
          if (!sub.ns.empty() && meta.get_string("namespace") != sub.ns) continue;
          if (!sub.fields.name_ok(meta.get_string("name"))) continue;
          if (!sub.sel.empty() && !selector_matches(sub.sel, *st.obj)) continue;
          std::string line = "{\"type\":\"ADDED\",\"object\":";
          if (meta_only) dump_partial_metadata(*st.obj, line);
          else st.obj->dump_to(line);
          line += "}\n";
          initial.push_back(std::make_shared<const std::string>(std::move(line)));
        }
      } else if (from < ts.compacted_rv) {
        gone = true;
      } else {
        auto it = std::upper_bound(ts.history.begin(), ts.history.end(), from,
                                   [](uint64_t v, const std::shared_ptr<const EventRec>& e) { return v < e->rv; });
        for (; it != ts.history.end(); ++it) {
          const auto& e = *it;
          if (e->type_key != sub.type_key) continue;
          if (!sub.ns.empty() && e->ns != sub.ns) continue;
          if (!sub.fields.name_ok(e->meta->get("metadata").get_string("name"))) continue;
          View view;
          if (!view_for(sub.sel, *e, &view)) continue;
          if (view == View::AsIs && !meta_only) initial.push_back(e->line);
          else initial.push_back(std::make_shared<const std::string>(e->line_as(view, meta_only)));
        }
      }
      if (!gone) {
        std::lock_guard<std::mutex> wg(ts.watches_mu);
        ts.watches.insert(subp);
      }
    }
    if (!w.start_chunked(200, "application/json")) {
      std::lock_guard<std::mutex> wg(ts.watches_mu);
      ts.watches.erase(subp);
      return;
    }
    if (gone) {
      Value ev = Value::object({{"type", "ERROR"},
                                {"object", status_body(410, "Expired", "too old resource version: " + rv_s + " (" +
                                                                           rv_str(compacted) + ")")}});
      w.write_chunk(ev.dump() + "\n");
      w.end_chunked();
      return;
    }
    bool ok = true;
    for (auto& l : initial) {
      if (!(ok = w.write_chunk(*l))) break;
    }
    if (ok && send_initial) {
      Value bm = Value::object(
          {{"type", "BOOKMARK"},
           {"object", Value::object({{"kind", p.ti->rt.kind},
                                     {"apiVersion", p.ti->rt.api_version()},
                                     {"metadata", Value::object({{"resourceVersion", rv_str(initial_rv)},
                                                                 {"annotations", Value::object({{"k8s.io/initial-events-end", "true"}})}})}})}});
      ok = w.write_chunk(bm.dump() + "\n");
    }
    auto deadline = std::chrono::steady_clock::now() + std::chrono::seconds(timeout_s);
    auto next_bookmark = std::chrono::steady_clock::now() + std::chrono::milliseconds(opts.bookmark_interval_ms);
    while (ok && !w.stopping()) {
      std::vector<QueuedEvent> batch;
      bool closed = false, overflow = false;
      {
        std::unique_lock<std::mutex> lk(sub.m);
        sub.cv.wait_for(lk, std::chrono::milliseconds(500), [&] { return !sub.q.empty() || sub.closed || sub.overflow; });
        const int coalesce_us = watch_coalesce_us.load(std::memory_order_relaxed);
        if (coalesce_us > 0 && !sub.q.empty() && sub.q.size() < 16 && !sub.closed) {
          sub.cv.wait_for(lk, std::chrono::microseconds(coalesce_us),
                          [&] { return sub.q.size() >= 16 || sub.closed || sub.overflow; });
        }
        batch.assign(sub.q.begin(), sub.q.end());
        sub.q.clear();
        closed = sub.closed;
        overflow = sub.overflow;
      }
      if (!batch.empty()) {
        std::string buf;
        for (auto& q : batch) buf += q.e->line_as(q.view, meta_only);
        const bool traced = trace::armed();
        if (traced) {
          for (auto& q : batch) trace::mark(q.e->meta->get("metadata").get_string("name"), trace_watch);
        }
        const int64_t w0 = metrics::now_ns();
        if (!w.write_chunk(buf)) break;
        const int64_t w1 = metrics::now_ns();
        stall::note_slow(slow_write, w0, w1);
        if (traced) {
          for (auto& q : batch) trace::mark_at(q.e->meta->get("metadata").get_string("name"), trace_written, w1);
        }
      }
      if (closed || overflow) break;
      auto now = std::chrono::steady_clock::now();
      if (now >= deadline) break;
      if (bookmarks && now >= next_bookmark) {
        uint64_t cur_rv;
        std::vector<QueuedEvent> pending;
        {
          SharedStoreLock lk(ts.seq, ts.seq_stats);
          cur_rv = rv.load();
          std::lock_guard<std::mutex> g(sub.m);
          pending.assign(sub.q.begin(), sub.q.end());
          sub.q.clear();
        }
        if (!pending.empty()) {
          std::string buf;
          for (auto& q : pending) buf += q.e->line_as(q.view, meta_only);
          if (!w.write_chunk(buf)) break;
        }
        Value bm = Value::object({{"type", "BOOKMARK"},
                                  {"object", Value::object({{"kind", p.ti->rt.kind},
                                                            {"apiVersion", p.ti->rt.api_version()},
                                                            {"metadata", Value::object({{"resourceVersion", rv_str(cur_rv)}})}})}});
        if (!w.write_chunk(bm.dump() + "\n")) break;
        next_bookmark = now + std::chrono::milliseconds(opts.bookmark_interval_ms);
      }
      if (batch.empty() && w.peer_closed()) break;
    }
    {
      std::lock_guard<std::mutex> wg(ts.watches_mu);
      ts.watches.erase(subp);
    }
    w.end_chunked();
  }

  void discovery(const std::string& path, http::ResponseWriter& w) {
    SharedStoreLock lk(types_mu, types_stats);
    if (path == "/api") {
      w.send_json(200, Value::object({{"kind", "APIVersions"}, {"versions", Value::array({"v1"})}}).dump());
      return;
    }
    if (path == "/apis") {
      std::map<std::string, std::set<std::string>> groups;
      for (auto& [k, ti] : types) {
        if (!ti.rt.group.empty()) groups[ti.rt.group].insert(ti.rt.version);
      }
      Value gl = Value::array();
      for (auto& [g, vs] : groups) {
        Value versions = Value::array();
        for (auto& v : vs) versions.push_back(Value::object({{"groupVersion", g + "/" + v}, {"version", v}}));
        gl.push_back(Value::object({{"name", g}, {"versions", versions}, {"preferredVersion", versions[0]}}));
      }
      w.send_json(200, Value::object({{"kind", "APIGroupList"}, {"apiVersion", "v1"}, {"groups", gl}}).dump());
      return;
    }
    std::string gv = path.rfind("/api/", 0) == 0 ? path.substr(5) : path.substr(6);
    Value res = Value::array();
    for (auto& [k, ti] : types) {
      if (ti.rt.api_version() != gv) continue;
      Value verbs = Value::array({"create", "delete", "get", "list", "patch", "update", "watch"});
      res.push_back(Value::object({{"name", ti.rt.plural}, {"namespaced", ti.rt.namespaced}, {"kind", ti.rt.kind}, {"verbs", verbs}}));
      if (ti.rt.has_status) {
        res.push_back(Value::object({{"name", ti.rt.plural + "/status"}, {"namespaced", ti.rt.namespaced}, {"kind", ti.rt.kind},
                                     {"verbs", Value::array({"get", "patch", "update"})}}));
      }
    }
    if (res.empty()) throw StatusError(404, "NotFound", "the server could not find the requested resource");
    w.send_json(200, Value::object({{"kind", "APIResourceList"}, {"apiVersion", "v1"}, {"groupVersion", gv}, {"resources", res}}).dump());
  }

  class HoldingWriter : public http::ResponseWriter {
   public:
    HoldingWriter(http::ResponseWriter& inner, int hold_ms)
        : ResponseWriter(nullptr, inner.keep_alive(), never_stops()), inner_(inner), hold_ms_(hold_ms) {}
    void send(int status, std::string_view body, const std::string& content_type,
              const http::Headers* extra) override {
      inner_.wait_stopping(std::chrono::milliseconds(hold_ms_));
      inner_.send(status, body, content_type, extra);
      sent_ = true;
      status_ = status;
    }
    bool start_chunked(int status, const std::string& content_type) override {
      sent_ = true;
      status_ = status;
      return inner_.start_chunked(status, content_type);
    }
    bool write_chunk(const std::string& data) override { return inner_.write_chunk(data); }
    void end_chunked() override { inner_.end_chunked(); }
    void abort() override { inner_.abort(); }
    bool peer_closed() override { return inner_.peer_closed(); }
    const char* protocol() const override { return inner_.protocol(); }

   private:
    static const CancelToken& never_stops() {
      static const CancelToken t;
      return t;
    }
    http::ResponseWriter& inner_;
    int hold_ms_;
  };

  bool inject_fault(const http::Request& req, http::ResponseWriter& w, int* hold_ms) {
    FaultRule hit;
    bool found = false;
    {
      std::lock_guard<std::mutex> lk(fault_mu);
      for (auto& f : faults) {
        if (f.remaining == 0) continue;
        if (!f.method.empty() && f.method != req.method) continue;
        std::string target = req.path + (req.query.empty() ? "" : "?" + req.query);
        if (!std::regex_search(target, f.path)) continue;
        if (f.remaining > 0) --f.remaining;
        hit = f;
        found = true;
        break;
      }
    }
    if (!found) return false;
    faults_hit.fetch_add(1);
    if (hit.delay_ms > 0 && w.wait_stopping(std::chrono::milliseconds(hit.delay_ms))) {
      w.abort();
      return true;
    }
    if (hit.reset) {
      w.abort();
      return true;
    }
    if (hit.hold_ms > 0 && hit.status <= 0) {
      *hold_ms = hit.hold_ms;
      return false;
    }
    if (hit.status > 0) {
      std::string reason = hit.status == 409   ? "Conflict"
                           : hit.status == 410 ? "Expired"
                           : hit.status == 429 ? "TooManyRequests"
                           : hit.status >= 500 ? "InternalError"
                                               : "BadRequest";
      http::Headers extra;
      if (hit.retry_after_s >= 0) extra.set("Retry-After", std::to_string(hit.retry_after_s));
      w.send(hit.status, status_body(hit.status, reason, hit.message.empty() ? "injected fault" : hit.message).dump(),
             "application/json", &extra);
      return true;
    }
    return false;
  }

  void control(http::Request& req, http::ResponseWriter& w) {
    if (req.path == "/_kl/faults" && req.method == "POST") {
      Value rules = json::parse(req.body);
      std::lock_guard<std::mutex> lk(fault_mu);
      if (req.query_param("append") != "true") faults.clear();
      for (const auto& r : rules.items()) {
        FaultRule f;
        f.method = r.get_string("method");
        f.path_src = r.get_string("path", ".*");
        f.path = std::regex(f.path_src);
        f.status = r.get("status").is_int() ? static_cast<int>(r.get("status").as_int()) : 0;
        f.delay_ms = r.get("delay_ms").is_int() ? static_cast<int>(r.get("delay_ms").as_int()) : 0;
        f.hold_ms = r.get("delay_response_ms").is_int() ? static_cast<int>(r.get("delay_response_ms").as_int()) : 0;
        f.remaining = r.get("count").is_int() ? static_cast<int>(r.get("count").as_int()) : -1;
        f.message = r.get_string("message");
        f.reset = r.get("reset").is_bool() && r.get("reset").as_bool();
        f.retry_after_s = r.get("retry_after").is_int() ? static_cast<int>(r.get("retry_after").as_int()) : -1;
        faults.push_back(std::move(f));
      }
      w.send_json(200, "{}");
      return;
    }
    if (req.path == "/_kl/faults" && req.method == "DELETE") {
      std::lock_guard<std::mutex> lk(fault_mu);
      faults.clear();
      w.send_json(200, "{}");
      return;
    }
    if (req.path == "/_kl/write-latency-us" && req.method == "POST") {
      try {
        size_t used = 0;
        const long long us = std::stoll(req.body, &used);
        if (us < 0 || us > 10000000) throw std::out_of_range("write latency");
        write_latency_us = us;
      } catch (const std::exception&) {
        w.send(400, "body must be 0..10000000 microseconds\n");
        return;
      }
      w.send(200, std::to_string(write_latency_us.load()) + "\n");
      return;
    }
    if (req.path == "/_kl/watch-coalesce-us" && req.method == "POST") {
      int prev = 0;
      try {
        size_t used = 0;
        const long us = std::stol(req.body, &used);
        if (us < 0 || us > 100000) throw std::out_of_range("watch coalesce");
        prev = watch_coalesce_us.exchange(static_cast<int>(us));
      } catch (const std::exception&) {
        w.send(400, "body must be 0..100000 microseconds\n");
        return;
      }
      w.send(200, std::to_string(prev) + "\n");
      return;
    }
    if (req.path == "/_kl/webhook-protocol" && req.method == "POST") {
      const bool h2 = req.body == "h2";
      if (!h2 && req.body != "http/1.1") {
        w.send(400, "body must be h2 or http/1.1\n");
        return;
      }
      {
        std::lock_guard<std::mutex> lk(hook_mu);
        webhook_h2 = h2;
        hook_fast.clear();
        hook_clients.clear();
      }
      w.send(200, h2 ? "h2\n" : "http/1.1\n");
      return;
    }
    if (req.path == "/_kl/compact" && req.method == "POST") {
      uint64_t at = 0;
      for_each_store([&](const std::string&, TypeStore& ts) {
        StoreLock lk(ts.seq, ts.seq_stats);
        at = rv.load();
        ts.compacted_rv = at;
        ts.history.clear();
      });
      w.send_json(200, Value::object({{"compacted_rv", static_cast<unsigned long long>(at)}}).dump());
      return;
    }
    if (req.path == "/_kl/drop-watches" && req.method == "POST") {
      size_t n = 0;
      for_each_store([&](const std::string&, TypeStore& ts) {
        std::lock_guard<std::mutex> wg(ts.watches_mu);
        n += ts.watches.size();
        for (const auto& ws : ts.watches) ws->close();
      });
      w.send_json(200, Value::object({{"dropped", static_cast<unsigned long long>(n)}}).dump());
      return;
    }
    if (req.path == "/_kl/stats") {
      Value counts = Value::object();
      Value locks = Value::object();
      size_t total = 0, n_watches = 0;
      uint64_t acq = 0, contended = 0, wait_ns = 0, hold_ns = 0;
      for_each_store([&](const std::string& key, TypeStore& ts) {
        {
          AllShards lk(ts, false);
          size_t n = 0;
          for (auto& sh : ts.shards) n += sh.objs.size();
          counts[key] = static_cast<unsigned long long>(n);
          total += n;
        }
        {
          std::lock_guard<std::mutex> wg(ts.watches_mu);
          n_watches += ts.watches.size();
        }
        auto account = [](const LockStats& st) {
          return Value::object({{"acquisitions", static_cast<unsigned long long>(st.acquisitions.load())},
                                {"contended", static_cast<unsigned long long>(st.contended.load())},
                                {"wait_ms", static_cast<double>(st.wait_ns.load()) * 1e-6},
                                {"hold_ms", static_cast<double>(st.hold_ns.load()) * 1e-6}});
        };
        for (const LockStats* st : {&ts.stats, &ts.seq_stats}) {
          acq += st->acquisitions.load();
          hold_ns += st->hold_ns.load();
          contended += st->contended.load();
          wait_ns += st->wait_ns.load();
        }
        const uint64_t a = ts.stats.acquisitions.load() + ts.seq_stats.acquisitions.load();
        if (a) {
          locks[key] = Value::object({{"acquisitions", static_cast<unsigned long long>(a)},
                                      {"hold_ms", static_cast<double>(ts.seq_stats.hold_ns.load()) * 1e-6},
                                      {"seq", account(ts.seq_stats)},
                                      {"shards", account(ts.stats)}});
        }
      });
      w.send_json(200, Value::object({{"resourceVersion", static_cast<unsigned long long>(rv.load())},
                                      {"objects", static_cast<unsigned long long>(total)},
                                      {"watches", static_cast<unsigned long long>(n_watches)},
                                      {"requests", static_cast<unsigned long long>(requests.load())},
                                      {"faults_hit", static_cast<unsigned long long>(faults_hit.load())},
                                      {"list_pages", static_cast<unsigned long long>(list_pages.load())},
                                      {"resource_version", rv_str(rv.load())},
                                      {"gc_collected", static_cast<unsigned long long>(gc_collected.load())},
                                      {"store_shards", static_cast<unsigned long long>(opts.store_shards)},
                                      {"gc_pending", static_cast<unsigned long long>([&] {
                                         std::lock_guard<std::mutex> g(gc_mu);
                                         return gc_queue.size();
                                       }())},
                                      {"store_lock", Value::object({
                                          {"acquisitions", static_cast<unsigned long long>(acq)},
                                          {"contended", static_cast<unsigned long long>(contended)},
                                          {"wait_ms", static_cast<double>(wait_ns) * 1e-6},
                                          {"hold_ms", static_cast<double>(hold_ns) * 1e-6}})},
                                      {"by_type_lock", locks},
                                      {"requests_by_kind", [&] {
                                         Value rq = Value::object();
                                         std::lock_guard<std::mutex> g(req_count_mu);
                                         for (auto& [k, v] : req_counts) rq[k] = static_cast<unsigned long long>(v);
                                         return rq;
                                       }()},
                                      {"by_type", counts}}).dump());
      return;
    }
    w.send(404, "not found\n");
  }

  std::mutex req_count_mu;
  std::map<std::string, uint64_t> req_counts;

  void handle(http::Request& req, http::ResponseWriter& w_conn) {
    http::ResponseWriter* wp = &w_conn;
    std::optional<HoldingWriter> holder;
    http::ResponseWriter& w_count = w_conn;
    requests.fetch_add(1, std::memory_order_relaxed);
    std::string res_key = "-";
    struct Count {
      Impl* im;
      const http::Request& req;
      http::ResponseWriter& w;
      std::string& res;
      ~Count() {
        std::string k = req.method + " " + res + " " + std::to_string(w.status_code());
        std::lock_guard<std::mutex> g(im->req_count_mu);
        im->req_counts[k]++;
      }
    } count{this, req, w_count, res_key};
    struct TraceSpan {
      int64_t t_recv = 0;
      ~TraceSpan() {
        if (!t_trace_tag.empty() && !t_trace_name.empty()) {
          trace::mark_at(t_trace_name, t_trace_tag + ".recv", t_recv);
          trace::mark(t_trace_name, t_trace_tag + ".resp");
        }
        t_trace_tag.clear();
        t_trace_name.clear();
      }
    } span;
    if (trace::armed()) span.t_recv = metrics::now_ns();
    try {
      int hold_ms = 0;
      if (inject_fault(req, w_conn, &hold_ms)) return;
      if (hold_ms > 0 && req.method != "GET") wp = &holder.emplace(w_conn, hold_ms);
      http::ResponseWriter& w = *wp;
      UserInfo user = authenticate(req);
      if (req.path == "/apis/authentication.k8s.io/v1/selfsubjectreviews" && req.method == "POST") {
        Value ui = Value::object({{"username", user.username}});
        if (!user.uid.empty()) ui["uid"] = user.uid;
        Value groups = Value::array();
        for (const auto& g : user.groups) groups.push_back(g);
        ui["groups"] = groups;
        w.send_json(201, Value::object({{"kind", "SelfSubjectReview"},
                                        {"apiVersion", "authentication.k8s.io/v1"},
                                        {"metadata", Value::object({{"creationTimestamp", Value()}})},
                                        {"status", Value::object({{"userInfo", ui}})}}).dump());
        return;
      }
      if (req.path == "/api" || req.path == "/apis") {
        discovery(req.path, w);
        return;
      }
      ParsedPath p;
      std::string group, version;
      std::vector<std::string> rest;
      if (!parse_path(req.path, p, group, version, rest)) {
        discovery(req.path, w);
        return;
      }
      res_key = p.ti->rt.plural + (p.sub.empty() ? "" : "/" + p.sub);
      if (p.collection && req.method == "GET") {
        std::string wq = req.query_param("watch");
        if (wq == "1" || wq == "true") res_key += " watch";
      }
      if (span.t_recv && req.method != "GET") {
        t_trace_tag = "kl." + res_key + "." + req.method + "." + field_manager(req, "unknown");
        t_trace_name = p.name;
      }
      if (!p.sub.empty() && p.sub != "status") throw StatusError(404, "NotFound", "subresource not supported: " + p.sub);
      if (!p.sub.empty() && !p.ti->rt.has_status) throw StatusError(404, "NotFound", "the server could not find the requested resource");
      const std::string& m = req.method;
      if (const int64_t lat = write_latency_us.load(std::memory_order_relaxed); lat > 0 && m != "GET") {
        std::this_thread::sleep_for(std::chrono::microseconds(lat));
      }
      if (p.collection) {
        if (m == "GET") {
          std::string wq = req.query_param("watch");
          if (wq == "1" || wq == "true") do_watch(p, req, w);
          else do_list(p, req, w);
        } else if (m == "POST") {
          do_create(p, req, user, w);
        } else {
          throw StatusError(405, "MethodNotAllowed", "method not allowed");
        }
        return;
      }
      if (m == "GET") do_get(p, w, wants_metadata(req));
      else if (m == "PUT") do_update(p, req, user, w);
      else if (m == "PATCH") do_patch(p, req, user, w);
      else if (m == "DELETE") do_delete(p, req, user, w);
      else throw StatusError(405, "MethodNotAllowed", "method not allowed");
    } catch (const StatusError& e) {
      if (!wp->sent()) wp->send_json(e.code, status_body(e.code, e.reason, e.what(), e.details).dump());
    } catch (const std::exception& e) {
      if (!wp->sent()) wp->send_json(500, status_body(500, "InternalError", e.what()).dump());
    }
  }
};

ApiServer::ApiServer(Options o) : impl_(std::make_unique<Impl>(std::move(o))) {}
ApiServer::~ApiServer() { stop(); }

void ApiServer::start() {
  http::ServerOptions so;
  so.addr = impl_->opts.addr;
  so.port = impl_->opts.port;
  so.name = "apiserver";
  so.idle_timeout_ms = 300000;
  if (!impl_->opts.tls_cert_file.empty()) {
    so.tls = net::TlsContext::server_from_files(
        impl_->opts.tls_cert_file, impl_->opts.tls_key_file,
        impl_->opts.client_ca_file.empty() ? "" : net::read_file(impl_->opts.client_ca_file));
  }
  impl_->server = std::make_unique<http::Server>(so);
  Impl* im = impl_.get();
  metrics::set_debug_endpoints(true);
  http::add_standard_routes(*impl_->server);
  impl_->server->handle("GET", "/healthz", [](http::Request&, http::ResponseWriter& w) { w.send(200, "ok"); });
  impl_->server->handle("GET", "/readyz", [](http::Request&, http::ResponseWriter& w) { w.send(200, "ok"); });
  impl_->server->handle("GET", "/livez", [](http::Request&, http::ResponseWriter& w) { w.send(200, "ok"); });
  impl_->server->handle("GET", "/version", [](http::Request&, http::ResponseWriter& w) {
    w.send_json(200, Value::object({{"major", "1"}, {"minor", "26"}, {"gitVersion", "v1.26.0-kube-lite"}, {"platform", "linux/amd64"}}).dump());
  });
  impl_->server->handle_prefix("/api", [im](http::Request& r, http::ResponseWriter& w) { im->handle(r, w); });
  impl_->server->handle_prefix("/_kl/", [im](http::Request& r, http::ResponseWriter& w) { im->control(r, w); });
  impl_->server->start();
}

uint16_t ApiServer::port() const { return impl_->server ? impl_->server->port() : 0; }

void ApiServer::stop() {
  if (impl_ && impl_->server) {
    impl_->for_each_store([](const std::string&, TypeStore& ts) {
      std::lock_guard<std::mutex> wg(ts.watches_mu);
      for (const auto& ws : ts.watches) ws->close();
    });
    impl_->server->stop(std::chrono::milliseconds(2000));
    impl_->server.reset();
  }
}

}
```

native/core/json.cc:

```cpp
#include "core/json.h"

#include <cctype>

#include <algorithm>
#include <charconv>
#include <cmath>
#include <cstring>
#include <numeric>

namespace bgc::json {

const Value kNull;

const char* type_name(Type t) {
  switch (t) {
    case Type::Null: return "null";
    case Type::Bool: return "boolean";
    case Type::Int:
    case Type::UInt: return "integer";
    case Type::Double: return "number";
    case Type::String: return "string";
    case Type::Array: return "array";
    case Type::Object: return "object";
  }
  return "?";
}

Value Value::array(std::initializer_list<Value> items) {
  Value v = array();
  v.arr_.assign(items.begin(), items.end());
  return v;
}

Value Value::object(std::initializer_list<std::pair<std::string, Value>> items) {
  Value v = object();
  v.keys_.reserve(items.size());
  v.arr_.reserve(items.size());
  for (auto& kv : items) v.set(kv.first, kv.second);
  return v;
}

void Value::set_unsigned(unsigned long long v) {
  if (v <= static_cast<unsigned long long>(INT64_MAX)) {
    type_ = Type::Int;
    num_.i = static_cast<int64_t>(v);
  } else {
    type_ = Type::UInt;
    num_.u = v;
  }
}

void Value::require(Type t, const char* what) const {
  if (type_ != t) {
    throw TypeError(std::string(what) + ": expected " + type_name(t) + ", got " +
                    type_name(type_));
  }
}

void Value::require_object(const char* what) {
  if (type_ == Type::Null) {
    type_ = Type::Object;
    return;
  }
  require(Type::Object, what);
}

bool Value::as_bool() const {
  require(Type::Bool, "as_bool");
  return num_.b;
}

int64_t Value::as_int() const {
  if (type_ == Type::Int) return num_.i;
  if (type_ == Type::UInt) throw TypeError("as_int: value out of int64 range");
  if (type_ == Type::Double) {
    double d = num_.d;
    if (std::floor(d) == d && d >= -9.2e18 && d <= 9.2e18) return static_cast<int64_t>(d);
  }
  throw TypeError(std::string("as_int: expected integer, got ") + type_name(type_));
}

uint64_t Value::as_uint() const {
  if (type_ == Type::UInt) return num_.u;
  if (type_ == Type::Int && num_.i >= 0) return static_cast<uint64_t>(num_.i);
  throw TypeError(std::string("as_uint: expected unsigned integer, got ") + type_name(type_));
}

double Value::as_double() const {
  switch (type_) {
    case Type::Int: return static_cast<double>(num_.i);
    case Type::UInt: return static_cast<double>(num_.u);
    case Type::Double: return num_.d;
    default: throw TypeError(std::string("as_double: expected number, got ") + type_name(type_));
  }
}

const std::string& Value::as_string() const {
  require(Type::String, "as_string");
  return str_;
}

std::string& Value::as_string_mut() {
  require(Type::String, "as_string_mut");
  return str_;
}

size_t Value::size() const {
  if (type_ == Type::Array || type_ == Type::Object) return arr_.size();
  return 0;
}

const Value& Value::operator[](size_t i) const {
  require(Type::Array, "index");
  if (i >= arr_.size()) throw TypeError("index out of range");
  return arr_[i];
}

Value& Value::operator[](size_t i) {
  require(Type::Array, "index");
  if (i >= arr_.size()) throw TypeError("index out of range");
  return arr_[i];
}

void Value::push_back(Value v) {
  if (type_ == Type::Null) type_ = Type::Array;
  require(Type::Array, "push_back");
  arr_.push_back(std::move(v));
}

const std::vector<Value>& Value::items() const {
  static const std::vector<Value> kEmpty;
  if (type_ != Type::Array && type_ != Type::Object) return kEmpty;
  return arr_;
}

std::vector<Value>& Value::items_mut() {
  if (type_ != Type::Array && type_ != Type::Object) {
    throw TypeError(std::string("items_mut on ") + type_name(type_));
  }
  return arr_;
}

void Value::erase_index(size_t i) {
  require(Type::Array, "erase_index");
  if (i >= arr_.size()) throw TypeError("index out of range");
  arr_.erase(arr_.begin() + static_cast<long>(i));
}

void Value::insert_at(size_t i, Value v) {
  require(Type::Array, "insert_at");
  if (i > arr_.size()) throw TypeError("index out of range");
  arr_.insert(arr_.begin() + static_cast<long>(i), std::move(v));
}

const Value* Value::find(std::string_view key) const {
  if (type_ != Type::Object) return nullptr;
  for (size_t i = 0; i < keys_.size(); ++i) {
    if (keys_[i] == key) return &arr_[i];
  }
  return nullptr;
}

Value* Value::find_mut(std::string_view key) {
  return const_cast<Value*>(static_cast<const Value*>(this)->find(key));
}

Value& Value::operator[](std::string_view key) {
  require_object("operator[]");
  for (size_t i = 0; i < keys_.size(); ++i) {
    if (keys_[i] == key) return arr_[i];
  }
  if (keys_.capacity() == 0) {
    keys_.reserve(4);
    arr_.reserve(4);
  }
  keys_.emplace_back(key);
  arr_.emplace_back();
  return arr_.back();
}

const Value& Value::at(std::string_view key) const {
  const Value* v = find(key);
  if (!v) throw TypeError("missing key: " + std::string(key));
  return *v;
}

const Value& Value::get(std::string_view key) const {
  const Value* v = find(key);
  return v ? *v : kNull;
}

void Value::set(std::string_view key, Value v) { (*this)[key] = std::move(v); }

bool Value::erase(std::string_view key) {
  if (type_ != Type::Object) return false;
  for (size_t i = 0; i < keys_.size(); ++i) {
    if (keys_[i] == key) {
      keys_.erase(keys_.begin() + static_cast<long>(i));
      arr_.erase(arr_.begin() + static_cast<long>(i));
      return true;
    }
  }
  return false;
}

const std::vector<std::string>& Value::keys() const {
  static const std::vector<std::string> kEmpty;
  return type_ == Type::Object ? keys_ : kEmpty;
}

void Value::sort_keys_recursive() {
  if (type_ == Type::Object) {
    std::vector<size_t> idx(keys_.size());
    std::iota(idx.begin(), idx.end(), 0);
    std::stable_sort(idx.begin(), idx.end(), [&](size_t a, size_t b) { return keys_[a] < keys_[b]; });
    std::vector<std::string> nk;
    std::vector<Value> nv;
    nk.reserve(idx.size());
    nv.reserve(idx.size());
    for (size_t i : idx) {
      nk.push_back(std::move(keys_[i]));
      nv.push_back(std::move(arr_[i]));
    }
    keys_ = std::move(nk);
    arr_ = std::move(nv);
  }
  if (type_ == Type::Object || type_ == Type::Array) {
    for (auto& v : arr_) v.sort_keys_recursive();
  }
}

const Value* Value::path(std::initializer_list<std::string_view> keys) const {
  const Value* cur = this;
  for (auto k : keys) {
    cur = cur->find(k);
    if (!cur) return nullptr;
  }
  return cur;
}

std::string Value::get_string(std::string_view key, const std::string& dflt) const {
  const Value* v = find(key);
  if (!v || !v->is_string()) return dflt;
  return v->str_;
}

bool Value::operator==(const Value& o) const {
  if (is_number() && o.is_number()) {
    if (type_ == Type::Double || o.type_ == Type::Double) return as_double() == o.as_double();
    if (type_ == Type::UInt || o.type_ == Type::UInt) {
      if (type_ != o.type_) return false;
      return num_.u == o.num_.u;
    }
    return num_.i == o.num_.i;
  }
  if (type_ != o.type_) return false;
  switch (type_) {
    case Type::Null: return true;
    case Type::Bool: return num_.b == o.num_.b;
    case Type::String: return str_ == o.str_;
    case Type::Array: return arr_ == o.arr_;
    case Type::Object: {
      if (keys_.size() != o.keys_.size()) return false;
      for (size_t i = 0; i < keys_.size(); ++i) {
        const Value* ov = o.find(keys_[i]);
        if (!ov || !(arr_[i] == *ov)) return false;
      }
      return true;
    }
    default: return false;
  }
}


void escape_string(std::string_view s, std::string& out) {
  static const char kHex[] = "0123456789abcdef";
  out.push_back('"');
  size_t run = 0;
  for (size_t i = 0; i < s.size(); ++i) {
    unsigned char c = static_cast<unsigned char>(s[i]);
    const char* rep = nullptr;
    char buf[7];
    if (c == '"') rep = "\\\"";
    else if (c == '\\') rep = "\\\\";
    else if (c == '\n') rep = "\\n";
    else if (c == '\r') rep = "\\r";
    else if (c == '\t') rep = "\\t";
    else if (c == '\b') rep = "\\b";
    else if (c == '\f') rep = "\\f";
    else if (c < 0x20) {
      buf[0] = '\\'; buf[1] = 'u'; buf[2] = '0'; buf[3] = '0';
      buf[4] = kHex[c >> 4]; buf[5] = kHex[c & 15]; buf[6] = 0;
      rep = buf;
    }
    if (rep) {
      out.append(s.data() + i - run, run);
      run = 0;
      out.append(rep);
    } else {
      ++run;
    }
  }
  out.append(s.data() + s.size() - run, run);
  out.push_back('"');
}

std::string quote(std::string_view s) {
  std::string out;
  out.reserve(s.size() + 2);
  escape_string(s, out);
  return out;
}

static void dump_double(double d, std::string& out) {
  if (!std::isfinite(d)) {
    out.append("null");
    return;
  }
  char buf[64];
  auto res = std::to_chars(buf, buf + sizeof(buf), d);
  std::string_view sv(buf, static_cast<size_t>(res.ptr - buf));
  out.append(sv);
  if (sv.find_first_of(".eEn") == std::string_view::npos) out.append(".0");
}

static void dump_impl(const Value& v, std::string& out, int indent, int depth);

void Value::dump_to(std::string& out) const { dump_impl(*this, out, -1, 0); }

std::string Value::dump() const {
  std::string out;
  out.reserve(128);
  dump_to(out);
  return out;
}

std::string Value::dump_pretty(int indent) const {
  std::string out;
  dump_impl(*this, out, indent, 0);
  return out;
}

static void newline_indent(std::string& out, int indent, int depth) {
  out.push_back('\n');
  out.append(static_cast<size_t>(indent * depth), ' ');
}

static void dump_impl(const Value& v, std::string& out, int indent, int depth) {
  char buf[32];
  switch (v.type()) {
    case Type::Null: out.append("null"); break;
    case Type::Bool: out.append(v.as_bool() ? "true" : "false"); break;
    case Type::Int: {
      auto r = std::to_chars(buf, buf + sizeof(buf), v.as_int());
      out.append(buf, static_cast<size_t>(r.ptr - buf));
      break;
    }
    case Type::UInt: {
      auto r = std::to_chars(buf, buf + sizeof(buf), v.as_uint());
      out.append(buf, static_cast<size_t>(r.ptr - buf));
      break;
    }
    case Type::Double: dump_double(v.as_double(), out); break;
    case Type::String: escape_string(v.as_string(), out); break;
    case Type::Array: {
      const auto& items = v.items();
      out.push_back('[');
      if (items.empty()) {
        out.push_back(']');
        break;
      }
      for (size_t i = 0; i < items.size(); ++i) {
        if (i) out.push_back(',');
        if (indent >= 0) newline_indent(out, indent, depth + 1);
        dump_impl(items[i], out, indent, depth + 1);
      }
      if (indent >= 0) newline_indent(out, indent, depth);
      out.push_back(']');
      break;
    }
    case Type::Object: {
      const auto& keys = v.keys();
      const auto& vals = v.values();
      out.push_back('{');
      if (keys.empty()) {
        out.push_back('}');
        break;
      }
      for (size_t i = 0; i < keys.size(); ++i) {
        if (i) out.push_back(',');
        if (indent >= 0) newline_indent(out, indent, depth + 1);
        escape_string(keys[i], out);
        out.push_back(':');
        if (indent >= 0) out.push_back(' ');
        dump_impl(vals[i], out, indent, depth + 1);
      }
      if (indent >= 0) newline_indent(out, indent, depth);
      out.push_back('}');
      break;
    }
  }
}


static thread_local std::vector<Value> t_stage_vals;
static thread_local std::vector<std::string> t_stage_keys;

class Parser {
 public:
  explicit Parser(std::string_view t, std::string_view drop_key = {})
      : s_(t), drop_key_(drop_key), vals_(t_stage_vals), keys_(t_stage_keys) {
    vals_.clear();
    keys_.clear();
  }
  ~Parser() {
    vals_.clear();
    keys_.clear();
    if (vals_.capacity() > 4096) std::vector<Value>().swap(vals_);
    if (keys_.capacity() > 4096) std::vector<std::string>().swap(keys_);
  }

  Value parse_document() {
    Value v;
    skip_ws();
    parse_value(v, 0);
    skip_ws();
    if (p_ != s_.size()) fail("trailing characters");
    return v;
  }

  Value parse_document(const Projection& root) {
    Value v;
    skip_ws();
    parse_projected(v, 0, &root);
    skip_ws();
    if (p_ != s_.size()) fail("trailing characters");
    return v;
  }

 private:
  [[noreturn]] void fail(const std::string& msg) const {
    size_t line = 1, col = 1;
    for (size_t i = 0; i < p_ && i < s_.size(); ++i) {
      if (s_[i] == '\n') {
        ++line;
        col = 1;
      } else {
        ++col;
      }
    }
    throw ParseError(msg, line, col);
  }

  void skip_ws() {
    while (p_ < s_.size()) {
      char c = s_[p_];
      if (c == ' ' || c == '\n' || c == '\r' || c == '\t') ++p_;
      else break;
    }
  }

  void expect_lit(const char* lit) {
    size_t n = std::strlen(lit);
    if (s_.substr(p_, n) != lit) fail("expected value");
    p_ += n;
  }

  void parse_value(Value& out, int depth) {
    if (depth > 512) fail("recursion limit exceeded");
    if (p_ >= s_.size()) fail("EOF while parsing a value");
    char c = s_[p_];
    switch (c) {
      case 'n': expect_lit("null"); out = Value(); return;
      case 't': expect_lit("true"); out = Value(true); return;
      case 'f': expect_lit("false"); out = Value(false); return;
      case '"': {
        out.type_ = Type::String;
        parse_string(out.str_);
        return;
      }
      case '[': {
        ++p_;
        out.type_ = Type::Array;
        skip_ws();
        if (p_ < s_.size() && s_[p_] == ']') {
          ++p_;
          return;
        }
        const size_t base = vals_.size();
        while (true) {
          skip_ws();
          Value child;
          parse_value(child, depth + 1);
          vals_.push_back(std::move(child));
          skip_ws();
          if (p_ >= s_.size()) fail("EOF while parsing a list");
          if (s_[p_] == ',') {
            ++p_;
            continue;
          }
          if (s_[p_] == ']') {
            ++p_;
            out.arr_.reserve(vals_.size() - base);
            for (size_t i = base; i < vals_.size(); ++i) out.arr_.push_back(std::move(vals_[i]));
            vals_.resize(base);
            return;
          }
          fail("expected `,` or `]`");
        }
      }
      case '{': {
        ++p_;
        out.type_ = Type::Object;
        skip_ws();
        if (p_ < s_.size() && s_[p_] == '}') {
          ++p_;
          return;
        }
        const size_t base = vals_.size();
        const size_t kbase = keys_.size();
        while (true) {
          skip_ws();
          if (p_ >= s_.size() || s_[p_] != '"') fail("key must be a string");
          std::string key;
          parse_string(key);
          skip_ws();
          if (p_ >= s_.size() || s_[p_] != ':') fail("expected `:`");
          ++p_;
          skip_ws();
          if (!drop_key_.empty() && key == drop_key_) {
            skip_value();
            skip_ws();
            if (p_ >= s_.size()) fail("EOF while parsing an object");
            if (s_[p_] == ',') {
              ++p_;
              continue;
            }
            if (s_[p_] != '}') fail("expected `,` or `}`");
            ++p_;
            finish_object(out, base, kbase);
            return;
          }
          Value child;
          parse_value(child, depth + 1);
          bool dup = false;
          for (size_t i = kbase; i < keys_.size(); ++i) {
            if (keys_[i] == key) {
              vals_[base + (i - kbase)] = std::move(child);
              dup = true;
              break;
            }
          }
          if (!dup) {
            keys_.push_back(std::move(key));
            vals_.push_back(std::move(child));
          }
          skip_ws();
          if (p_ >= s_.size()) fail("EOF while parsing an object");
          if (s_[p_] == ',') {
            ++p_;
            continue;
          }
          if (s_[p_] == '}') {
            ++p_;
            finish_object(out, base, kbase);
            return;
          }
          fail("expected `,` or `}`");
        }
      }
      default:
        if (c == '-' || (c >= '0' && c <= '9')) {
          parse_number(out);
          return;
        }
        fail("expected value");
    }
  }

  void parse_projected(Value& out, int depth, const Projection* p) {
    if (p && p->mode == Projection::Keep) {
      parse_value(out, depth);
      return;
    }
    if (!p || p->mode == Projection::Shape || p_ >= s_.size() || s_[p_] != '{') {
      if (p && p->mode == Projection::Descend) {
        parse_value(out, depth);
        return;
      }
      shape_value(out, depth);
      return;
    }
    if (depth > 512) fail("recursion limit exceeded");
    ++p_;
    out.type_ = Type::Object;
    skip_ws();
    if (p_ < s_.size() && s_[p_] == '}') {
      ++p_;
      return;
    }
    const size_t base = vals_.size();
    const size_t kbase = keys_.size();
    while (true) {
      skip_ws();
      if (p_ >= s_.size() || s_[p_] != '"') fail("key must be a string");
      std::string key;
      parse_string(key);
      skip_ws();
      if (p_ >= s_.size() || s_[p_] != ':') fail("expected `:`");
      ++p_;
      skip_ws();
      const Projection* child = nullptr;
      for (size_t i = 0; i < p->n_children; ++i) {
        if (p->children[i].key == key) {
          child = &p->children[i];
          break;
        }
      }
      if (!child && p->omit_unnamed) {
        skip_value();
        skip_ws();
        if (p_ >= s_.size()) fail("EOF while parsing an object");
        if (s_[p_] == ',') {
          ++p_;
          continue;
        }
        if (s_[p_] == '}') {
          ++p_;
          finish_object(out, base, kbase);
          return;
        }
        fail("expected `,` or `}`");
      }
      Value v;
      parse_projected(v, depth + 1, child);
      bool dup = false;
      for (size_t i = kbase; i < keys_.size(); ++i) {
        if (keys_[i] == key) {
          vals_[base + (i - kbase)] = std::move(v);
          dup = true;
          break;
        }
      }
      if (!dup) {
        keys_.push_back(std::move(key));
        vals_.push_back(std::move(v));
      }
      skip_ws();
      if (p_ >= s_.size()) fail("EOF while parsing an object");
      if (s_[p_] == ',') {
        ++p_;
        continue;
      }
      if (s_[p_] == '}') {
        ++p_;
        finish_object(out, base, kbase);
        return;
      }
      fail("expected `,` or `}`");
    }
  }

  void shape_value(Value& out, int depth) {
    if (depth > 512) fail("recursion limit exceeded");
    if (p_ >= s_.size()) fail("EOF while parsing a value");
    const char c = s_[p_];
    if (c == '"') {
      static thread_local std::string scratch;
      parse_string(scratch);
      out = Value(std::string());
      return;
    }
    if (c == '[' || c == '{') {
      const bool obj = c == '{';
      ++p_;
      out = obj ? Value::object() : Value::array();
      skip_ws();
      if (p_ < s_.size() && s_[p_] == (obj ? '}' : ']')) {
        ++p_;
        return;
      }
      while (true) {
        skip_ws();
        if (obj) {
          if (p_ >= s_.size() || s_[p_] != '"') fail("key must be a string");
          static thread_local std::string key;
          parse_string(key);
          skip_ws();
          if (p_ >= s_.size() || s_[p_] != ':') fail("expected `:`");
          ++p_;
          skip_ws();
        }
        Value child;
        shape_value(child, depth + 1);
        skip_ws();
        if (p_ >= s_.size()) fail(obj ? "EOF while parsing an object" : "EOF while parsing a list");
        if (s_[p_] == ',') {
          ++p_;
          continue;
        }
        if (s_[p_] == (obj ? '}' : ']')) {
          ++p_;
          return;
        }
        fail(obj ? "expected `,` or `}`" : "expected `,` or `]`");
      }
    }
    parse_value(out, depth);
    if (out.is_number()) out = Value(0);
    else if (out.is_bool()) out = Value(false);
  }

  static int hexval(char c) {
    if (c >= '0' && c <= '9') return c - '0';
    if (c >= 'a' && c <= 'f') return c - 'a' + 10;
    if (c >= 'A' && c <= 'F') return c - 'A' + 10;
    return -1;
  }

  uint32_t parse_hex4() {
    if (p_ + 4 > s_.size()) fail("EOF while parsing a string");
    uint32_t v = 0;
    for (int i = 0; i < 4; ++i) {
      int h = hexval(s_[p_ + static_cast<size_t>(i)]);
      if (h < 0) fail("invalid escape");
      v = (v << 4) | static_cast<uint32_t>(h);
    }
    p_ += 4;
    return v;
  }

  static void append_utf8(uint32_t cp, std::string& out) {
    if (cp < 0x80) {
      out.push_back(static_cast<char>(cp));
    } else if (cp < 0x800) {
      out.push_back(static_cast<char>(0xC0 | (cp >> 6)));
      out.push_back(static_cast<char>(0x80 | (cp & 0x3F)));
    } else if (cp < 0x10000) {
      out.push_back(static_cast<char>(0xE0 | (cp >> 12)));
      out.push_back(static_cast<char>(0x80 | ((cp >> 6) & 0x3F)));
      out.push_back(static_cast<char>(0x80 | (cp & 0x3F)));
    } else {
      out.push_back(static_cast<char>(0xF0 | (cp >> 18)));
      out.push_back(static_cast<char>(0x80 | ((cp >> 12) & 0x3F)));
      out.push_back(static_cast<char>(0x80 | ((cp >> 6) & 0x3F)));
      out.push_back(static_cast<char>(0x80 | (cp & 0x3F)));
    }
  }

  void finish_object(Value& out, size_t base, size_t kbase) {
    const size_t n = keys_.size() - kbase;
    out.arr_.reserve(n);
    out.keys_.reserve(n);
    for (size_t i = 0; i < n; ++i) {
      out.keys_.push_back(std::move(keys_[kbase + i]));
      out.arr_.push_back(std::move(vals_[base + i]));
    }
    keys_.resize(kbase);
    vals_.resize(base);
  }

  void skip_string() {
    ++p_;
    while (p_ < s_.size()) {
      const char c = s_[p_];
      if (c == '\\') {
        p_ += 2;
      } else if (c == '"') {
        ++p_;
        return;
      } else {
        ++p_;
      }
    }
    fail("EOF while parsing a string");
  }

  void skip_value() {
    if (p_ >= s_.size()) fail("EOF while parsing a value");
    const char c = s_[p_];
    if (c == '"') {
      skip_string();
      return;
    }
    if (c == '{' || c == '[') {
      int nest = 0;
      while (p_ < s_.size()) {
        const char d = s_[p_];
        if (d == '"') {
          skip_string();
          continue;
        }
        if (d == '{' || d == '[') {
          if (++nest > 512) fail("recursion limit exceeded");
        } else if (d == '}' || d == ']') {
          if (--nest == 0) {
            ++p_;
            return;
          }
        }
        ++p_;
      }
      fail("EOF while parsing a value");
    }
    const size_t start = p_;
    while (p_ < s_.size()) {
      const char d = s_[p_];
      if (d == ',' || d == '}' || d == ']' || d == ' ' || d == '\n' || d == '\r' || d == '\t') break;
      ++p_;
    }
    if (p_ == start) fail("expected value");
  }

  void parse_string(std::string& out) {
    ++p_;
    out.clear();
    size_t start = p_;
    while (true) {
      while (p_ < s_.size()) {
        unsigned char c = static_cast<unsigned char>(s_[p_]);
        if (c == '"' || c == '\\' || c < 0x20) break;
        ++p_;
      }
      out.append(s_.data() + start, p_ - start);
      if (p_ >= s_.size()) fail("EOF while parsing a string");
      char c = s_[p_];
      if (c == '"') {
        ++p_;
        return;
      }
      if (static_cast<unsigned char>(c) < 0x20) fail("control character in string");
      ++p_;
      if (p_ >= s_.size()) fail("EOF while parsing a string");
      char e = s_[p_++];
      switch (e) {
        case '"': out.push_back('"'); break;
        case '\\': out.push_back('\\'); break;
        case '/': out.push_back('/'); break;
        case 'b': out.push_back('\b'); break;
        case 'f': out.push_back('\f'); break;
        case 'n': out.push_back('\n'); break;
        case 'r': out.push_back('\r'); break;
        case 't': out.push_back('\t'); break;
        case 'u': {
          uint32_t cp = parse_hex4();
          if (cp >= 0xD800 && cp <= 0xDBFF) {
            if (p_ + 6 <= s_.size() && s_[p_] == '\\' && s_[p_ + 1] == 'u') {
              p_ += 2;
              uint32_t lo = parse_hex4();
              if (lo < 0xDC00 || lo > 0xDFFF) fail("lone leading surrogate");
              cp = 0x10000 + ((cp - 0xD800) << 10) + (lo - 0xDC00);
            } else {
              fail("lone leading surrogate");
            }
          } else if (cp >= 0xDC00 && cp <= 0xDFFF) {
            fail("lone trailing surrogate");
          }
          append_utf8(cp, out);
          break;
        }
        default: fail("invalid escape");
      }
      start = p_;
    }
  }

  void parse_number(Value& out) {
    size_t start = p_;
    bool neg = false;
    if (s_[p_] == '-') {
      neg = true;
      ++p_;
    }
    if (p_ >= s_.size() || !(s_[p_] >= '0' && s_[p_] <= '9')) fail("invalid number");
    if (s_[p_] == '0' && p_ + 1 < s_.size() && s_[p_ + 1] >= '0' && s_[p_ + 1] <= '9') {
      fail("invalid number");
    }
    while (p_ < s_.size() && s_[p_] >= '0' && s_[p_] <= '9') ++p_;
    bool is_float = false;
    if (p_ < s_.size() && s_[p_] == '.') {
      is_float = true;
      ++p_;
      if (p_ >= s_.size() || !(s_[p_] >= '0' && s_[p_] <= '9')) fail("invalid number");
      while (p_ < s_.size() && s_[p_] >= '0' && s_[p_] <= '9') ++p_;
    }
    if (p_ < s_.size() && (s_[p_] == 'e' || s_[p_] == 'E')) {
      is_float = true;
      ++p_;
      if (p_ < s_.size() && (s_[p_] == '+' || s_[p_] == '-')) ++p_;
      if (p_ >= s_.size() || !(s_[p_] >= '0' && s_[p_] <= '9')) fail("invalid number");
      while (p_ < s_.size() && s_[p_] >= '0' && s_[p_] <= '9') ++p_;
    }
    const char* b = s_.data() + start;
    const char* e = s_.data() + p_;
    if (!is_float) {
      if (neg) {
        int64_t v;
        auto r = std::from_chars(b, e, v);
        if (r.ec == std::errc()) {
          out = Value(static_cast<long long>(v));
          return;
        }
      } else {
        uint64_t v;
        auto r = std::from_chars(b, e, v);
        if (r.ec == std::errc()) {
          out = Value(static_cast<unsigned long long>(v));
          return;
        }
      }
    }
    double d;
    auto r = std::from_chars(b, e, d);
    if (r.ec != std::errc() && r.ec != std::errc::result_out_of_range) fail("invalid number");
    out = Value(d);
  }

  std::string_view s_;
  std::string_view drop_key_;
  size_t p_ = 0;
  std::vector<Value>& vals_;
  std::vector<std::string>& keys_;
};

namespace {
size_t skip_string(std::string_view t, size_t i) {
  for (++i; i < t.size(); ++i) {
    if (t[i] == '\\') ++i;
    else if (t[i] == '"') return i + 1;
  }
  return t.size();
}
size_t skip_value(std::string_view t, size_t i) {
  if (i >= t.size()) return i;
  if (t[i] == '"') return skip_string(t, i);
  if (t[i] == '{' || t[i] == '[') {
    int depth = 0;
    for (; i < t.size(); ++i) {
      const char c = t[i];
      if (c == '"') {
        i = skip_string(t, i) - 1;
      } else if (c == '{' || c == '[') {
        ++depth;
      } else if (c == '}' || c == ']') {
        if (--depth == 0) return i + 1;
      }
    }
    return t.size();
  }
  while (i < t.size() && t[i] != ',' && t[i] != '}' && t[i] != ']' && !std::isspace(static_cast<unsigned char>(t[i]))) ++i;
  return i;
}
size_t skip_ws(std::string_view t, size_t i) {
  while (i < t.size() && std::isspace(static_cast<unsigned char>(t[i]))) ++i;
  return i;
}
}

std::string_view raw_member(std::string_view t, std::string_view key) {
  size_t i = skip_ws(t, 0);
  if (i >= t.size() || t[i] != '{') return {};
  ++i;
  while (true) {
    i = skip_ws(t, i);
    if (i >= t.size() || t[i] != '"') return {};
    const size_t k0 = i + 1, k1 = skip_string(t, i);
    const std::string_view k = t.substr(k0, k1 - 1 - k0);
    i = skip_ws(t, k1);
    if (i >= t.size() || t[i] != ':') return {};
    i = skip_ws(t, i + 1);
    const size_t v0 = i, v1 = skip_value(t, i);
    if (k == key) return t.substr(v0, v1 - v0);
    i = skip_ws(t, v1);
    if (i >= t.size() || t[i] != ',') return {};
    ++i;
  }
}

Value parse(std::string_view text) { return Parser(text).parse_document(); }
Value parse(std::string_view text, std::string_view drop_key) { return Parser(text, drop_key).parse_document(); }

Value parse_projected(std::string_view text, const Projection& root) { return Parser(text).parse_document(root); }

bool try_parse_projected(std::string_view text, const Projection& root, Value& out, std::string* err) {
  try {
    out = parse_projected(text, root);
    return true;
  } catch (const ParseError& e) {
    if (err) *err = e.what();
    return false;
  }
}

bool try_parse(std::string_view text, Value& out, std::string* err) {
  try {
    out = parse(text);
    return true;
  } catch (const ParseError& e) {
    if (err) *err = e.what();
    return false;
  }
}

}
```

Measured before the change: 10620.

## Cache rendered managedFields text and splice it into serialized objects

Managed field entries become shared, immutable entries that each cache their own JSON text. Objects store a marker in place of managedFields, and the cached text is spliced in whenever the object is serialized, so unchanged managers are not rebuilt on every commit. Admission review bodies reuse precomputed kind/resource and user JSON, and old objects are taken from the stored watch line. JSON string escaping switches to a lookup table. The cost is extra complexity: marker handling must be materialized before JSON patches touch managedFields, and any serialization path that skips the splice would emit the marker.

```diff
diff --git a/native/apiserver/server.cc b/native/apiserver/server.cc
--- a/native/apiserver/server.cc
+++ b/native/apiserver/server.cc
@@ -235,6 +235,7 @@
     v["groups"] = g;
     return v;
   }
+  std::string json_text;
 };
 
 struct TypeStore;
@@ -245,6 +246,14 @@
   bool custom = false;
   std::shared_ptr<TypeStore> store;
   std::string key() const { return rt.group + "/" + rt.version + "/" + rt.plural; }
+  std::string review_kind, review_request_kind;
+  void render_review_text() {
+    const std::string gv = "{\"group\":" + json::quote(rt.group) + ",\"version\":" + json::quote(rt.version);
+    const std::string gvk = gv + ",\"kind\":" + json::quote(rt.kind) + "}";
+    const std::string gvr = gv + ",\"resource\":" + json::quote(rt.plural) + "}";
+    review_kind = ",\"kind\":" + gvk + ",\"resource\":" + gvr;
+    review_request_kind = ",\"requestKind\":" + gvk + ",\"requestResource\":" + gvr;
+  }
 };
 
 struct ManagerEntry {
@@ -253,11 +262,53 @@
   std::string time;
   std::string subresource;
   FieldSet fields;
+  mutable std::string text;
   bool operator==(const ManagerEntry& o) const {
     return operation == o.operation && fields == o.fields && subresource == o.subresource;
   }
+  void render(const std::string& key, const std::string& default_api_version) const {
+    Value ent = Value::object({{"manager", key.substr(0, key.find('\x1f'))}, {"operation", operation},
+                               {"apiVersion", api_version.empty() ? default_api_version : api_version},
+                               {"time", time}, {"fieldsType", "FieldsV1"}, {"fieldsV1", fields_v1(fields)}});
+    if (!subresource.empty()) ent["subresource"] = subresource;
+    text = ent.dump();
+  }
 };
-using Managers = std::map<std::string, ManagerEntry>;
+using Managers = std::map<std::string, std::shared_ptr<const ManagerEntry>>;
+
+bool same_managers(const Managers& a, const Managers& b) {
+  if (a.size() != b.size()) return false;
+  for (auto ia = a.begin(), ib = b.begin(); ia != a.end(); ++ia, ++ib) {
+    if (ia->first != ib->first) return false;
+    if (ia->second != ib->second && !(*ia->second == *ib->second)) return false;
+  }
+  return true;
+}
+
+class ManagersEdit {
+ public:
+  explicit ManagersEdit(Managers& m) : m_(m) {}
+  ManagerEntry& entry(const std::string& key) {
+    auto it = open_.find(key);
+    if (it != open_.end()) return *it->second;
+    auto cur = m_.find(key);
+    auto e = cur != m_.end() ? std::make_shared<ManagerEntry>(*cur->second) : std::make_shared<ManagerEntry>();
+    e->text.clear();
+    open_[key] = e;
+    return *e;
+  }
+  void finish() {
+    for (auto& [key, e] : open_) {
+      if (e->fields.empty()) m_.erase(key);
+      else m_[key] = std::move(e);
+    }
+    open_.clear();
+  }
+
+ private:
+  Managers& m_;
+  std::map<std::string, std::shared_ptr<ManagerEntry>> open_;
+};
 
 inline const std::shared_ptr<const Managers>& no_managers() {
   static const std::shared_ptr<const Managers> empty = std::make_shared<const Managers>();
@@ -276,10 +327,82 @@
   return a && a->find("as=PartialObjectMetadata") != std::string::npos;
 }
 
-void dump_partial_metadata(const Value& obj, std::string& out) {
+const std::string& managed_marker() {
+  static const std::string m = "\x01mf\x01";
+  return m;
+}
+
+void set_managed_marker(Value& obj, const Managers& m) {
+  if (m.empty()) obj["metadata"].erase("managedFields");
+  else obj["metadata"]["managedFields"] = managed_marker();
+}
+
+void append_managed(const Managers& m, std::string& out) {
+  out += '[';
+  bool first = true;
+  for (const auto& [key, e] : m) {
+    if (!first) out += ',';
+    first = false;
+    out += e->text;
+  }
+  out += ']';
+}
+
+void splice_managed(std::string& out, size_t from, const Managers& m) {
+  static const std::string key = "\"managedFields\":";
+  static const std::string needle = key + Value(managed_marker()).dump();
+  const size_t pos = out.find(needle, from);
+  if (pos == std::string::npos) return;
+  std::string arr;
+  size_t n = 2;
+  for (const auto& [k, e] : m) n += e->text.size() + 1;
+  arr.reserve(n);
+  append_managed(m, arr);
+  out.replace(pos + key.size(), needle.size() - key.size(), arr);
+}
+
+void dump_stored(const Value& obj, const Managers& m, std::string& out) {
+  const size_t from = out.size();
+  obj.dump_to(out);
+  splice_managed(out, from, m);
+}
+
+std::string dump_stored(const Value& obj, const Managers& m) {
+  std::string out;
+  out.reserve(1024);
+  dump_stored(obj, m, out);
+  return out;
+}
+
+void dump_partial_metadata(const Value& obj, const Managers& m, std::string& out) {
   out += "{\"kind\":\"PartialObjectMetadata\",\"apiVersion\":\"meta.k8s.io/v1\",\"metadata\":";
+  const size_t from = out.size();
   obj.get("metadata").dump_to(out);
+  splice_managed(out, from, m);
   out += "}";
+}
+
+void materialize_managed(Value& obj, const Managers& m) {
+  Value* md = obj.find_mut("metadata");
+  Value* mf = md ? md->find_mut("managedFields") : nullptr;
+  if (!mf || !mf->is_string() || mf->as_string() != managed_marker()) return;
+  std::string text;
+  append_managed(m, text);
+  *mf = json::parse(text);
+}
+
+bool patch_touches_managed(const Value& patch) {
+  auto touches = [](const std::string& p) {
+    return p.empty() || p == "/metadata" || p.rfind("/metadata/managedFields", 0) == 0;
+  };
+  if (!patch.is_array()) return false;
+  for (const Value& op : patch.items()) {
+    for (const char* f : {"path", "from"}) {
+      const Value* v = op.find(f);
+      if (v && v->is_string() && touches(v->as_string())) return true;
+    }
+  }
+  return false;
 }
 
 std::string partial_metadata_line(const std::string& line) {
@@ -604,17 +727,24 @@
   if (!t_trace_tag.empty()) trace::mark(name, t_trace_tag + step);
 }
 
+std::string_view line_object(const std::string& line) {
+  static const std::string kObjectKey = ",\"object\":";
+  size_t at = line.find(kObjectKey);
+  if (at == std::string::npos || line.size() < at + kObjectKey.size() + 2) return {};
+  at += kObjectKey.size();
+  return std::string_view(line).substr(at, line.size() - at - 2);
+}
+
 struct WriteResult {
   std::shared_ptr<const Value> obj;
   int code = 200;
   std::shared_ptr<const std::string> line;
-  std::string_view body() const {
-    static const std::string kPrefixEnd = ",\"object\":";
-    if (!line) return {};
-    size_t at = line->find(kPrefixEnd);
-    if (at == std::string::npos || line->size() < at + kPrefixEnd.size() + 2) return {};
-    at += kPrefixEnd.size();
-    return std::string_view(*line).substr(at, line->size() - at - 2);
+  std::shared_ptr<const Managers> managers = no_managers();
+  std::string_view body() const { return line ? line_object(*line) : std::string_view(); }
+  void send(http::ResponseWriter& w) const {
+    const std::string_view b = body();
+    if (!b.empty()) w.send_json(code, b);
+    else w.send_json(code, dump_stored(*obj, *managers));
   }
 };
 
@@ -656,9 +786,14 @@
   std::mutex fault_mu;
   std::vector<FaultRule> faults;
 
+  struct ObjRef {
+    std::shared_ptr<const Value> obj;
+    std::shared_ptr<const Managers> managers;
+    const Value* operator->() const { return obj.get(); }
+  };
   struct ListSnapshot {
     uint64_t rv = 0;
-    std::vector<std::shared_ptr<const Value>> items;
+    std::vector<ObjRef> items;
     std::chrono::steady_clock::time_point expires;
   };
   std::mutex list_mu;
@@ -722,6 +857,7 @@
       TypeInfo ti;
       ti.rt = *rt;
       ti.store = std::make_shared<TypeStore>(opts.store_shards);
+      ti.render_review_text();
       types[ti.key()] = ti;
     }
     if (!opts.token_file.empty()) load_tokens(opts.token_file);
@@ -802,6 +938,7 @@
         while (std::getline(gs, g, ',')) u.groups.push_back(g);
       }
       u.groups.push_back("system:authenticated");
+      u.json_text = u.to_json().dump();
       tokens[cols[0]] = u;
     }
   }
@@ -896,7 +1033,8 @@
   }
 
   struct PreparedEvent {
-    std::string head, tail;
+    std::string line;
+    size_t rv_at = 0;
     bool ok = false;
     std::shared_ptr<const Value> filter;
     std::shared_ptr<EventRec> rec;
@@ -1061,7 +1199,9 @@
   }
 
   void call_webhooks(const TypeInfo& ti, const std::string& sub, const std::string& op, const std::string& ns,
-                     const std::string& name, Value* obj, const Value* old, const UserInfo& user) {
+                     const std::string& name, Value* obj, const Value* old,
+                     const std::shared_ptr<const std::string>& old_line, const Managers& old_managers,
+                     const UserInfo& user) {
     auto hooks = matching_webhooks(ti, sub, op);
     if (hooks.empty()) return;
     static auto& hist = metrics::Registry::global().histogram("kl_webhook_duration_seconds", "Webhook callout latency");
@@ -1076,32 +1216,44 @@
       std::string fail_policy = hook.get_string("failurePolicy", "Fail");
       int timeout_s = hook.get("timeoutSeconds").is_int() ? static_cast<int>(hook.get("timeoutSeconds").as_int()) : 10;
       std::string uid = crypto::uuid_v4();
-      const std::string opts_kind = op == "CREATE" ? "CreateOptions" : op == "DELETE" ? "DeleteOptions" : "UpdateOptions";
-      const std::string gvk = "{\"group\":" + json::quote(ti.rt.group) + ",\"version\":" + json::quote(ti.rt.version) +
-                              ",\"kind\":" + json::quote(ti.rt.kind) + "}";
-      const std::string gvr = "{\"group\":" + json::quote(ti.rt.group) + ",\"version\":" + json::quote(ti.rt.version) +
-                              ",\"resource\":" + json::quote(ti.rt.plural) + "}";
+      const char* const tail =
+          op == "CREATE" ? ",\"dryRun\":false,\"options\":{\"kind\":\"CreateOptions\",\"apiVersion\":\"meta.k8s.io/v1\"}}}"
+          : op == "DELETE" ? ",\"dryRun\":false,\"options\":{\"kind\":\"DeleteOptions\",\"apiVersion\":\"meta.k8s.io/v1\"}}}"
+                           : ",\"dryRun\":false,\"options\":{\"kind\":\"UpdateOptions\",\"apiVersion\":\"meta.k8s.io/v1\"}}}";
+      const std::string_view old_text = old && old_line ? line_object(*old_line) : std::string_view();
       std::string body;
-      body.reserve(1024 + (obj ? 2048 : 0) + (old ? 2048 : 0));
+      body.reserve(1024 + (obj ? 2048 : 0) + (old ? std::max<size_t>(2048, old_text.size()) : 0));
       body += "{\"kind\":\"AdmissionReview\",\"apiVersion\":\"admission.k8s.io/v1\",\"request\":{\"uid\":";
-      body += json::quote(uid);
-      body += ",\"kind\":" + gvk + ",\"resource\":" + gvr;
-      if (!sub.empty()) body += ",\"subResource\":" + json::quote(sub);
-      body += ",\"requestKind\":" + gvk + ",\"requestResource\":" + gvr;
-      if (!sub.empty()) body += ",\"requestSubResource\":" + json::quote(sub);
-      body += ",\"name\":" + json::quote(name);
-      if (!ns.empty()) body += ",\"namespace\":" + json::quote(ns);
-      body += ",\"operation\":" + json::quote(op);
+      json::escape_string(uid, body);
+      body += ti.review_kind;
+      if (!sub.empty()) {
+        body += ",\"subResource\":";
+        json::escape_string(sub, body);
+      }
+      body += ti.review_request_kind;
+      if (!sub.empty()) {
+        body += ",\"requestSubResource\":";
+        json::escape_string(sub, body);
+      }
+      body += ",\"name\":";
+      json::escape_string(name, body);
+      if (!ns.empty()) {
+        body += ",\"namespace\":";
+        json::escape_string(ns, body);
+      }
+      body += ",\"operation\":";
+      json::escape_string(op, body);
       body += ",\"userInfo\":";
-      user.to_json().dump_to(body);
+      if (!user.json_text.empty()) body += user.json_text;
+      else user.to_json().dump_to(body);
       body += ",\"object\":";
-      if (obj) obj->dump_to(body);
+      if (obj) dump_stored(*obj, old_managers, body);
       else body += "null";
       body += ",\"oldObject\":";
-      if (old) old->dump_to(body);
-      else body += "null";
-      body += ",\"dryRun\":false,\"options\":{\"kind\":" + json::quote(opts_kind) +
-              ",\"apiVersion\":\"meta.k8s.io/v1\"}}}";
+      if (!old) body += "null";
+      else if (!old_text.empty()) body.append(old_text);
+      else dump_stored(*old, old_managers, body);
+      body += tail;
       std::string err;
       Value resp_review;
       int64_t t0 = metrics::now_ns();
@@ -1157,6 +1309,7 @@
           throw StatusError(500, "InternalError", "invalid patch from webhook " + hm.name + ": " + perr);
         }
         try {
+          if (patch_touches_managed(patch)) materialize_managed(*obj, old_managers);
           json::apply_patch(*obj, patch);
         } catch (const std::exception& e) {
           throw StatusError(500, "InternalError",
@@ -1231,6 +1384,7 @@
       }
       ti.schema = schema;
       ti.store = std::make_shared<TypeStore>(opts.store_shards);
+      ti.render_review_text();
       types[ti.key()] = ti;
     }
   }
@@ -1278,21 +1432,6 @@
     if (obj.get("spec").get("finalizers").empty()) return;
     obj["spec"]["finalizers"] = Value::array();
     commit_locked(*nti, "", name, std::move(obj), *it->second.managers, &it->second);
-  }
-
-  static void render_managed(Value& obj, const Managers& m, const std::string& api_version) {
-    Value arr = Value::array();
-    for (const auto& [key, e] : m) {
-      if (e.fields.empty()) continue;
-      std::string mgr = key.substr(0, key.find('\x1f'));
-      Value ent = Value::object({{"manager", mgr}, {"operation", e.operation},
-                                 {"apiVersion", e.api_version.empty() ? api_version : e.api_version},
-                                 {"time", e.time}, {"fieldsType", "FieldsV1"}, {"fieldsV1", fields_v1(e.fields)}});
-      if (!e.subresource.empty()) ent["subresource"] = e.subresource;
-      arr.push_back(std::move(ent));
-    }
-    if (arr.empty()) obj["metadata"].erase("managedFields");
-    else obj["metadata"]["managedFields"] = std::move(arr);
   }
 
   static bool same_content(const Value& a, const Value& b) {
@@ -1348,12 +1487,21 @@
     FieldSet changed, removed;
     if (status_write) diff_member_leaves(before, after, "status", changed, removed);
     else diff_leaves(before, after, changed, removed);
-    for (auto& [name, e] : m) {
+    ManagersEdit edit(m);
+    for (const auto& [name, cur] : m) {
+      auto owns = [&cur = *cur](const FieldSet& paths) {
+        for (const auto& p : paths) {
+          if (cur.fields.count(p)) return true;
+        }
+        return false;
+      };
+      if (!owns(changed) && !owns(removed)) continue;
+      ManagerEntry& e = edit.entry(name);
       for (const auto& p : changed) e.fields.erase(p);
       for (const auto& p : removed) e.fields.erase(p);
     }
     if (!changed.empty()) {
-      auto& e = m[status_write ? manager + "\x1fstatus" : manager];
+      ManagerEntry& e = edit.entry(status_write ? manager + "\x1fstatus" : manager);
       if (e.operation.empty()) {
         e.operation = "Update";
         e.api_version = api_version;
@@ -1365,39 +1513,43 @@
       if (status_write) e.subresource = "status";
       for (const auto& p : changed) e.fields.insert(p);
     }
-    for (auto it = m.begin(); it != m.end();) {
-      if (it->second.fields.empty()) it = m.erase(it);
-      else ++it;
-    }
+    edit.finish();
   }
 
   static const std::string& rv_placeholder() {
     static const std::string p = "\x01rv\x01";
     return p;
   }
+  static const std::string& rv_placeholder_text() {
+    static const std::string t = Value(rv_placeholder()).dump();
+    return t;
+  }
   static PreparedEvent prepare_commit(Value& obj, const Managers& managers, const std::string& api_version,
                                       const char* type) {
     obj["metadata"]["resourceVersion"] = rv_placeholder();
-    render_managed(obj, managers, api_version);
+    for (const auto& [key, e] : managers) {
+      if (e->text.empty()) e->render(key, api_version);
+    }
+    set_managed_marker(obj, managers);
     std::string line = std::string("{\"type\":\"") + type + "\",\"object\":";
-    obj.dump_to(line);
+    line.reserve(2048);
+    dump_stored(obj, managers, line);
     line += "}\n";
-    static const std::string needle = "\"resourceVersion\":" + Value(rv_placeholder()).dump();
+    static const std::string needle = "\"resourceVersion\":" + rv_placeholder_text();
     PreparedEvent pe;
     pe.filter = filter_view(obj);
     pe.rec = std::make_shared<EventRec>();
     size_t pos = line.find(needle);
     if (pos == std::string::npos) return pe;
-    pe.head.assign(line, 0, pos);
-    pe.head += "\"resourceVersion\":\"";
-    pe.tail.assign(line, pos + needle.size() - 1, std::string::npos);
+    pe.rv_at = pos + needle.size() - rv_placeholder_text().size() + 1;
+    pe.line = std::move(line);
     pe.ok = true;
     return pe;
   }
 
   std::shared_ptr<const Value> commit_locked(const TypeInfo& ti, const std::string& ns, const std::string& name,
                                             Value obj, Managers managers, const Stored* prev,
-                                            const PreparedEvent* pe = nullptr, bool* dangling = nullptr,
+                                            PreparedEvent* pe = nullptr, bool* dangling = nullptr,
                                             std::shared_ptr<const std::string>* line_out = nullptr) {
     TypeStore& ts = *ti.store;
     PreparedEvent local;
@@ -1429,7 +1581,7 @@
         t->prev_line = std::move(held);
       } else {
         std::string l = "{\"type\":\"MODIFIED\",\"object\":";
-        prev->obj->dump_to(l);
+        dump_stored(*prev->obj, *prev->managers, l);
         l += "}\n";
         t->prev_line = std::make_shared<const std::string>(std::move(l));
       }
@@ -1444,14 +1596,13 @@
       digits = rv_str(new_rv);
       std::string preline;
       if (pe->ok) {
-        preline.reserve(pe->head.size() + digits.size() + pe->tail.size());
-        preline += pe->head;
-        preline += digits;
-        preline += pe->tail;
+        pe->line.replace(pe->rv_at, rv_placeholder_text().size() - 2, digits);
+        preline = std::move(pe->line);
+        pe->ok = false;
       } else {
         obj["metadata"]["resourceVersion"] = digits;
         preline = std::string("{\"type\":\"") + (prev ? "MODIFIED" : "ADDED") + "\",\"object\":";
-        obj.dump_to(preline);
+        dump_stored(obj, managers, preline);
         preline += "}\n";
       }
       line = emit_locked(ti, ns, new_rv, std::move(preline), pe->filter ? pe->filter : filter_view(obj), std::move(rec));
@@ -1486,14 +1637,11 @@
     std::shared_ptr<const Value> ptr = it->second.obj;
     std::string line = "{\"type\":\"DELETED\",\"object\":";
     const size_t obj_at = line.size();
-    static const std::string kObjectKey = ",\"object\":";
     const std::shared_ptr<const std::string> held = it->second.line.lock();
-    const std::string* committed = held.get();
-    const size_t at = committed ? committed->find(kObjectKey) : std::string::npos;
-    if (at != std::string::npos && committed->size() >= at + kObjectKey.size() + 2) {
-      line.append(*committed, at + kObjectKey.size(), committed->size() - (at + kObjectKey.size()) - 2);
+    if (const std::string_view committed = held ? line_object(*held) : std::string_view(); !committed.empty()) {
+      line.append(committed);
     } else {
-      ptr->dump_to(line);
+      dump_stored(*ptr, *it->second.managers, line);
     }
     line += "}\n";
     const std::string old_rv = "\"resourceVersion\":" + json::quote(ptr->get("metadata").get_string("resourceVersion"));
@@ -1526,7 +1674,7 @@
         Value final_obj = *ptr;
         final_obj["metadata"]["resourceVersion"] = digits;
         line = "{\"type\":\"DELETED\",\"object\":";
-        final_obj.dump_to(line);
+        dump_stored(final_obj, *it->second.managers, line);
         line += "}\n";
       }
       emit_locked(ti, ns, new_rv, std::move(line), std::move(filter), nullptr);
@@ -1653,19 +1801,20 @@
                                                                      {"field", "metadata.namespace"}})})}}));
         }
       }
-      if (exists && same_content(obj, *cur_copy.obj) && managers == *cur_copy.managers) {
-        return {cur_copy.obj, 200, nullptr};
+      if (exists && same_content(obj, *cur_copy.obj) && same_managers(managers, *cur_copy.managers)) {
+        return {cur_copy.obj, 200, nullptr, cur_copy.managers};
       }
       trace_step(name, ".hook0");
-      call_webhooks(ti, sub, op, ns, name, &obj, exists ? cur_copy.obj.get() : nullptr, user);
+      call_webhooks(ti, sub, op, ns, name, &obj, exists ? cur_copy.obj.get() : nullptr,
+                    exists ? cur_copy.line.lock() : nullptr, *cur_copy.managers, user);
       trace_step(name, ".hook1");
       obj["metadata"]["name"] = name;
       if (ti.rt.namespaced) obj["metadata"]["namespace"] = ns;
       else obj["metadata"].erase("namespace");
       canonicalize_quantities(ti, obj);
       validate_object(ti, name, ns, obj);
-      if (exists && same_content(obj, *cur_copy.obj) && managers == *cur_copy.managers) {
-        return {cur_copy.obj, 200, nullptr};
+      if (exists && same_content(obj, *cur_copy.obj) && same_managers(managers, *cur_copy.managers)) {
+        return {cur_copy.obj, 200, nullptr, cur_copy.managers};
       }
       if (exists && spec_changed(*cur_copy.obj, obj)) {
         int64_t gen = cur_copy.obj->get("metadata").get("generation").is_int()
@@ -1682,7 +1831,7 @@
         if (obj.get("metadata").contains("deletionTimestamp") && obj.get("metadata").get("finalizers").empty() &&
             !(is_core_namespaces(ti) && opts.namespace_termination && !obj.get("spec").get("finalizers").empty())) {
           erase_locked(ti, ns, name);
-          return {cur_copy.obj, 200, nullptr};
+          return {cur_copy.obj, 200, nullptr, cur_copy.managers};
         }
         (void)is_status;
         WriteResult wr;
@@ -1782,11 +1931,7 @@
                        return {std::move(obj), std::move(m)};
                      },
                      true, false);
-    {
-      std::string_view b = res.body();
-      if (!b.empty()) w.send_json(res.code, b);
-      else w.send_json(res.code, res.obj->dump());
-    }
+    res.send(w);
   }
 
   void do_update(ParsedPath& p, const http::Request& req, const UserInfo& user, http::ResponseWriter& w) {
@@ -1823,11 +1968,7 @@
                        return {std::move(obj), std::move(m)};
                      },
                      false, is_status);
-    {
-      std::string_view b = res.body();
-      if (!b.empty()) w.send_json(res.code, b);
-      else w.send_json(res.code, res.obj->dump());
-    }
+    res.send(w);
   }
 
   std::pair<Value, Managers> apply_ssa(const TypeInfo& ti, const Stored* cur, const Value& config,
@@ -1856,7 +1997,7 @@
       const Value* want = get_path(config, f);
       const Value* have = get_path(live, f);
       for (auto& [other, e] : m) {
-        if (other == manager || !e.fields.count(f)) continue;
+        if (other == manager || !e->fields.count(f)) continue;
         if (have && want && *have == *want) continue;
         conflicts.emplace_back(other, f);
       }
@@ -1871,15 +2012,17 @@
       }
       throw StatusError(409, "Conflict", msg);
     }
-    if (force) {
-      for (const auto& [other, f] : conflicts) m[other].fields.erase(f);
+    if (force && !conflicts.empty()) {
+      ManagersEdit edit(m);
+      for (const auto& [other, f] : conflicts) edit.entry(other).fields.erase(f);
+      edit.finish();
     }
     if (auto it = m.find(manager); it != m.end()) {
-      for (const auto& f : it->second.fields) {
+      for (const auto& f : it->second->fields) {
         if (cfg_fields.count(f)) continue;
         bool other_owner = false;
         for (auto& [other, e] : m) {
-          if (other != manager && e.fields.count(f)) other_owner = true;
+          if (other != manager && e->fields.count(f)) other_owner = true;
         }
         if (!other_owner) remove_path(live, f);
       }
@@ -1887,15 +2030,15 @@
     for (const auto& f : cfg_fields) {
       if (const Value* v = get_path(config, f)) set_path(live, f, *v);
     }
-    auto& me = m[manager];
-    me.operation = "Apply";
-    me.api_version = ti.rt.api_version();
-    me.time = now_rfc3339();
-    me.subresource = is_status ? "status" : "";
-    me.fields = cfg_fields;
-    for (auto it = m.begin(); it != m.end();) {
-      if (it->second.fields.empty()) it = m.erase(it);
-      else ++it;
+    {
+      ManagersEdit edit(m);
+      ManagerEntry& me = edit.entry(manager);
+      me.operation = "Apply";
+      me.api_version = ti.rt.api_version();
+      me.time = now_rfc3339();
+      me.subresource = is_status ? "status" : "";
+      me.fields = std::move(cfg_fields);
+      edit.finish();
     }
     if (cur && ti.rt.has_status && !is_status) {
       if (cur->obj->contains("status")) live["status"] = cur->obj->get("status");
@@ -1926,6 +2069,7 @@
                        Value obj = *cur->obj;
                        try {
                          if (ct.find("json-patch") != std::string::npos) {
+                           if (patch_touches_managed(patch)) materialize_managed(obj, *cur->managers);
                            json::apply_patch(obj, patch);
                          } else {
                            json::apply_merge_patch(obj, patch);
@@ -1954,15 +2098,13 @@
                        return {std::move(obj), std::move(m)};
                      },
                      is_apply, is_status);
-    {
-      std::string_view b = res.body();
-      if (!b.empty()) w.send_json(res.code, b);
-      else w.send_json(res.code, res.obj->dump());
-    }
+    res.send(w);
   }
 
   void do_delete(ParsedPath& p, const http::Request& req, const UserInfo& user, http::ResponseWriter& w) {
     std::shared_ptr<const Value> cur;
+    std::shared_ptr<const Managers> cur_managers;
+    std::weak_ptr<const std::string> cur_line;
     const std::string key = obj_key(p.ti->rt, p.ns, p.name);
     auto& sh = p.ti->store->shard(key);
     {
@@ -1970,9 +2112,11 @@
       auto it = sh.objs.find(key);
       if (it == sh.objs.end()) throw not_found(p.ti->rt, p.name);
       cur = it->second.obj;
+      cur_managers = it->second.managers;
+      cur_line = it->second.line;
     }
     trace_step(p.name, ".hook0");
-    call_webhooks(*p.ti, "", "DELETE", p.ns, p.name, nullptr, cur.get(), user);
+    call_webhooks(*p.ti, "", "DELETE", p.ns, p.name, nullptr, cur.get(), cur_line.lock(), *cur_managers, user);
     trace_step(p.name, ".hook1");
     StoreLock lk(sh.mu, p.ti->store->stats);
     auto it = sh.objs.find(key);
@@ -1981,7 +2125,7 @@
     if (is_core_namespaces(*p.ti) && opts.namespace_termination) {
       auto ptr = meta.contains("deletionTimestamp") ? it->second.obj
                                                     : terminate_namespace_locked(*p.ti, p.name, it->second);
-      w.send_json(200, ptr->dump());
+      w.send_json(200, dump_stored(*ptr, *it->second.managers));
       return;
     }
     if (!meta.get("finalizers").empty()) {
@@ -1990,10 +2134,10 @@
         obj["metadata"]["deletionTimestamp"] = now_rfc3339();
         obj["metadata"]["deletionGracePeriodSeconds"] = 0;
         auto ptr = commit_locked(*p.ti, p.ns, p.name, std::move(obj), *it->second.managers, &it->second);
-        w.send_json(202, ptr->dump());
+        w.send_json(202, dump_stored(*ptr, *it->second.managers));
         return;
       }
-      w.send_json(202, it->second.obj->dump());
+      w.send_json(202, dump_stored(*it->second.obj, *it->second.managers));
       return;
     }
     erase_locked(*p.ti, p.ns, p.name);
@@ -2003,6 +2147,7 @@
 
   void do_get(ParsedPath& p, http::ResponseWriter& w, bool meta_only = false) {
     std::shared_ptr<const Value> obj;
+    std::shared_ptr<const Managers> managers;
     {
       const std::string key = obj_key(p.ti->rt, p.ns, p.name);
       auto& sh = p.ti->store->shard(key);
@@ -2010,20 +2155,21 @@
       auto it = sh.objs.find(key);
       if (it == sh.objs.end()) throw not_found(p.ti->rt, p.name);
       obj = it->second.obj;
+      managers = it->second.managers;
     }
     if (meta_only) {
       std::string out;
-      dump_partial_metadata(*obj, out);
+      dump_partial_metadata(*obj, *managers, out);
       w.send_json(200, out);
       return;
     }
-    w.send_json(200, obj->dump());
+    w.send_json(200, dump_stored(*obj, *managers));
   }
 
   void do_list(ParsedPath& p, const http::Request& req, http::ResponseWriter& w) {
     const int64_t limit = req.has_query_param("limit") ? std::atoll(req.query_param("limit").c_str()) : 0;
     const std::string cont = req.query_param("continue");
-    std::vector<std::shared_ptr<const Value>> items;
+    std::vector<ObjRef> items;
     uint64_t list_rv = 0;
     size_t offset = 0;
     uint64_t snap_id = 0;
@@ -2054,7 +2200,7 @@
           if (!ff.name_ok(meta.get_string("name"))) continue;
           if (!ff.ns.empty() && meta.get_string("namespace") != ff.ns) continue;
           if (!sel.empty() && !selector_matches(sel, *st.obj)) continue;
-          items.push_back(st.obj);
+          items.push_back({st.obj, st.managers});
         }
       }
       std::sort(items.begin(), items.end(), [](const auto& a, const auto& b) {
@@ -2095,8 +2241,8 @@
     out += "},\"items\":[";
     for (size_t i = offset; i < end; ++i) {
       if (i != offset) out.push_back(',');
-      if (meta_only) dump_partial_metadata(*items[i], out);
-      else items[i]->dump_to(out);
+      if (meta_only) dump_partial_metadata(*items[i].obj, *items[i].managers, out);
+      else dump_stored(*items[i].obj, *items[i].managers, out);
     }
     out += "]}";
     w.send_json(200, out);
@@ -2151,8 +2297,8 @@
           if (!sub.fields.name_ok(meta.get_string("name"))) continue;
           if (!sub.sel.empty() && !selector_matches(sub.sel, *st.obj)) continue;
           std::string line = "{\"type\":\"ADDED\",\"object\":";
-          if (meta_only) dump_partial_metadata(*st.obj, line);
-          else st.obj->dump_to(line);
+          if (meta_only) dump_partial_metadata(*st.obj, *st.managers, line);
+          else dump_stored(*st.obj, *st.managers, line);
           line += "}\n";
           initial.push_back(std::make_shared<const std::string>(std::move(line)));
         }
diff --git a/native/core/json.cc b/native/core/json.cc
--- a/native/core/json.cc
+++ b/native/core/json.cc
@@ -273,35 +273,46 @@
 }
 
 
+namespace {
+
+struct EscapeTable {
+  char cls[256] = {};
+  constexpr EscapeTable() {
+    for (int c = 0; c < 0x20; ++c) cls[c] = 'u';
+    cls[static_cast<unsigned char>('"')] = '"';
+    cls[static_cast<unsigned char>('\\')] = '\\';
+    cls[static_cast<unsigned char>('\n')] = 'n';
+    cls[static_cast<unsigned char>('\r')] = 'r';
+    cls[static_cast<unsigned char>('\t')] = 't';
+    cls[static_cast<unsigned char>('\b')] = 'b';
+    cls[static_cast<unsigned char>('\f')] = 'f';
+  }
+};
+constexpr EscapeTable kEscape;
+
+}
+
 void escape_string(std::string_view s, std::string& out) {
   static const char kHex[] = "0123456789abcdef";
+  const char* const p = s.data();
+  const size_t n = s.size();
   out.push_back('"');
-  size_t run = 0;
-  for (size_t i = 0; i < s.size(); ++i) {
-    unsigned char c = static_cast<unsigned char>(s[i]);
-    const char* rep = nullptr;
-    char buf[7];
-    if (c == '"') rep = "\\\"";
-    else if (c == '\\') rep = "\\\\";
-    else if (c == '\n') rep = "\\n";
-    else if (c == '\r') rep = "\\r";
-    else if (c == '\t') rep = "\\t";
-    else if (c == '\b') rep = "\\b";
-    else if (c == '\f') rep = "\\f";
-    else if (c < 0x20) {
-      buf[0] = '\\'; buf[1] = 'u'; buf[2] = '0'; buf[3] = '0';
-      buf[4] = kHex[c >> 4]; buf[5] = kHex[c & 15]; buf[6] = 0;
-      rep = buf;
-    }
-    if (rep) {
-      out.append(s.data() + i - run, run);
-      run = 0;
-      out.append(rep);
+  size_t start = 0;
+  for (size_t i = 0; i < n; ++i) {
+    const unsigned char c = static_cast<unsigned char>(p[i]);
+    const char cls = kEscape.cls[c];
+    if (cls == 0) continue;
+    out.append(p + start, i - start);
+    start = i + 1;
+    if (cls == 'u') {
+      const char buf[6] = {'\\', 'u', '0', '0', kHex[c >> 4], kHex[c & 15]};
+      out.append(buf, 6);
     } else {
-      ++run;
-    }
-  }
-  out.append(s.data() + s.size() - run, run);
+      const char buf[2] = {'\\', cls};
+      out.append(buf, 2);
+    }
+  }
+  out.append(p + start, n - start);
   out.push_back('"');
 }
 
```

Measured after the change: 10480. 0.986x the previous value.
